# dscripka/openWakeWord

Measured on AMD Instinct MI355X. Metric: real-time audio frames/sec (80 ms frame, 3 wakewords), whole job; real-time streams = value/12.5, higher is better.
Workload: dtype f32 as 3xf16 split MFMA, fp32 accumulate; 1 GPU; 131072 concurrent 16 kHz streams per GPU x 3 heads (alexa,hey_mycroft,hey_jarvis), 80 ms frames, BASELINE configs[3] per-GPU shard; streams_per_gpu=131072, frame_samples=1280, collective=none, gather=none, rccl_ranks=0, pcm_distribution=Gaussian, RMS 3000, pcm=resident in HBM, kernels=mfma_rr_f16x3, graph=False, vad=off, weights=synthetic seed 1234, step_blocks=1

## Files before the change

openwakeword_amd/csrc/owwhip.hip:

```cpp
#include <hip/hip_runtime.h>

#include <algorithm>
#include <cmath>
#include <cstdio>
#include <cstdlib>
#include <cstring>
#include <ctime>
#include <exception>
#include <mutex>
#include <new>
#include <unordered_map>
#include <dlfcn.h>
#include <string>
#include <vector>

#include "owwhip.h"
#include "owwhip_pack.h"
#include "owwhip_ingest.h"
#include "owwhip_mem.h"
#include "owwhip_masked_host.h"
#include "owwhip_bank_host.h"
#include "owwhip_verifier_host.h"
#include "owwhip_state_host.h"
#include "owwhip_postproc.h"
#include "owwhip_kernels.h"
#include "owwhip_rr.h"
#include "owwhip_hx.h"
#include "owwhip_vad.h"
#include "owwhip_fused.h"
#include "owwhip_state.h"
#include "owwhip_events.h"
#include "owwhip_audio.h"
#include "owwhip_dense.h"
#include "owwhip_dense_hits_host.h"

using namespace owk;
using namespace owp;
using owm::DevBuf;
using owm::PinnedBuf;

namespace {

#define OWW_GUARD_BEGIN try {
#define OWW_GUARD_END                                                                                              \
    } catch (const std::bad_alloc&) { return fail(OWW_ENOMEM, "%s: out of host memory", __func__);                 \
    } catch (const std::exception& e__) { return fail(OWW_ESTATE, "%s: unexpected C++ exception: %s", __func__, e__.what()); \
    } catch (...) { return fail(OWW_ESTATE, "%s: unexpected C++ exception", __func__); }

#define HIPCHK(expr)                                                                         \
    do {                                                                                     \
        hipError_t e__ = (expr);                                                             \
        if (e__ != hipSuccess) return fail(OWW_EHIP, "%s failed: %s", #expr, hipGetErrorString(e__)); \
    } while (0)

struct GuardRange { char* base; size_t reserve, mapped; hipMemGenericAllocationHandle_t hnd; };
std::mutex g_guard_mu;
std::unordered_map<void*, GuardRange> g_guard;
int guard_mode() {
    static const int mode = [] { const char* e = getenv("OWW_GUARD_ALLOC"); return e ? atoi(e) : 0; }();
    return mode;
}
hipError_t guard_alloc(void** p, size_t n, int line) {
    int dev = 0;
    hipError_t e = hipGetDevice(&dev);
    if (e != hipSuccess) return e;
    hipMemAllocationProp prop = {};
    prop.type = hipMemAllocationTypePinned;
    prop.location.type = hipMemLocationTypeDevice;
    prop.location.id = dev;
    size_t gran = 0;
    if ((e = hipMemGetAllocationGranularity(&gran, &prop, hipMemAllocationGranularityMinimum)) != hipSuccess) return e;
    GuardRange g{};
    g.mapped = (std::max<size_t>(n, 1) + gran - 1) / gran * gran;
    g.reserve = g.mapped + 2 * gran;
    void* base = nullptr;
    if ((e = hipMemAddressReserve(&base, g.reserve, gran, nullptr, 0)) != hipSuccess) return e;
    g.base = static_cast<char*>(base);
    if ((e = hipMemCreate(&g.hnd, g.mapped, &prop, 0)) != hipSuccess) { (void)hipMemAddressFree(base, g.reserve); return e; }
    hipMemAccessDesc acc = {};
    acc.location = prop.location;
    acc.flags = hipMemAccessFlagsProtReadWrite;
    if ((e = hipMemMap(g.base + gran, g.mapped, 0, g.hnd, 0)) != hipSuccess ||
        (e = hipMemSetAccess(g.base + gran, g.mapped, &acc, 1)) != hipSuccess) {
        (void)hipMemRelease(g.hnd); (void)hipMemAddressFree(base, g.reserve); return e;
    }
    char* user = guard_mode() == 2 ? g.base + gran : g.base + gran + g.mapped - (n + 15) / 16 * 16;
    fprintf(stderr, "[owwhip guard] line %d: %zu bytes at [%p, %p), mapped [%p, %p)\n", line, n, (void*)user, (void*)(user + n),
            (void*)(g.base + gran), (void*)(g.base + gran + g.mapped));
    std::lock_guard<std::mutex> lk(g_guard_mu);
    g_guard[user] = g;
    *p = user;
    return hipSuccess;
}
hipError_t dev_alloc(void** p, size_t n, int line) {
    if (!guard_mode()) return hipMalloc(p, n);
    return guard_alloc(p, n, line);
}
hipError_t dev_free(void* p) {
    if (!guard_mode() || !p) return hipFree(p);
    GuardRange g;
    {
        std::lock_guard<std::mutex> lk(g_guard_mu);
        auto it = g_guard.find(p);
        if (it == g_guard.end()) return hipFree(p);
        g = it->second;
        g_guard.erase(it);
    }
    (void)hipDeviceSynchronize();
    const size_t gran = (g.reserve - g.mapped) / 2;
    (void)hipMemUnmap(g.base + gran, g.mapped);
    (void)hipMemRelease(g.hnd);
    return hipMemAddressFree(g.base, g.reserve);
}
}

namespace owm {
int dev_alloc_raw(void** p, size_t bytes, int line) { return dev_alloc(p, bytes, line); }
int dev_free_raw(void* p) { return dev_free(p); }
int pinned_alloc_raw(void** p, size_t bytes, unsigned flags) { return hipHostMalloc(p, bytes, flags); }
int pinned_free_raw(void* p) { return hipHostFree(p); }
int event_create_raw(hipEvent_t* e, unsigned flags) { return hipEventCreateWithFlags(e, flags); }
int event_destroy_raw(hipEvent_t e) { return hipEventDestroy(e); }
int stream_create_raw(hipStream_t* s, unsigned flags) { return hipStreamCreateWithFlags(s, flags); }
int stream_destroy_raw(hipStream_t s) { return hipStreamDestroy(s); }
}

namespace {
inline hipError_t herr(int e) { return static_cast<hipError_t>(e); }

hipError_t guard_copy(void* dst, const void* src, size_t n, hipMemcpyKind kind, hipStream_t st) {
    PinnedBuf<char> pin;
    hipError_t e = herr(pin.alloc(n, hipHostMallocDefault));
    if (e != hipSuccess) return e;
    if (kind == hipMemcpyHostToDevice) {
        memcpy(pin, src, n);
        e = hipMemcpyAsync(dst, pin, n, kind, st);
        if (e == hipSuccess) e = hipStreamSynchronize(st);
    } else {
        e = hipMemcpyAsync(pin, src, n, kind, st);
        if (e == hipSuccess) e = hipStreamSynchronize(st);
        if (e == hipSuccess) memcpy(dst, pin, n);
    }
    return e;
}
inline hipError_t copy_async(void* dst, const void* src, size_t n, hipMemcpyKind kind, hipStream_t st) {
    if (guard_mode() && n && (kind == hipMemcpyHostToDevice || kind == hipMemcpyDeviceToHost)) return guard_copy(dst, src, n, kind, st);
    return hipMemcpyAsync(dst, src, n, kind, st);
}
inline hipError_t copy_sync(void* dst, const void* src, size_t n, hipMemcpyKind kind) {
    if (guard_mode() && n && (kind == hipMemcpyHostToDevice || kind == hipMemcpyDeviceToHost)) return guard_copy(dst, src, n, kind, nullptr);
    const hipError_t e = hipMemcpy(dst, src, n, kind);
    return e != hipSuccess || kind != hipMemcpyHostToDevice ? e : hipStreamSynchronize(nullptr);
}

constexpr int kSmallLaunchWgs = 2 * 256;
constexpr int kResidentBMinGroups = 8192;
constexpr int kResidentBWgs = 256;

struct FastGroup : HeadGroup {
    DevBuf<NetDesc> d_nets;
    const float* d_w1pk = nullptr;
    const float* d_b1cat = nullptr;
    const float* d_w1hx = nullptr;
    std::vector<owh::HeadHxNet> hx_net;
};

owh::HeadHxNet make_hx_net(const NetHost& n, int ht, const HxNetPack& p, const float* img, const float* b3, int hx_efeat) {
    const int HP = 16 * ht;
    const float* pd = img + p.pad;
    owh::HeadHxNet o{};
    o.w2hx = img + p.w2; o.b1 = pd; o.ln1g = pd + HP; o.ln1b = pd + 2 * HP; o.b2 = pd + 3 * HP; o.ln2g = pd + 4 * HP; o.ln2b = pd + 5 * HP;
    if (ht == 4) { o.w3 = pd + 6 * HP; o.b3 = b3 ? b3 : pd + 7 * HP; }
    else { o.b3 = pd + 6 * HP; o.w3hx = img + p.w3; o.u3 = std::ldexp(1.0f, -p.e3); }
    o.has_ln = n.has_ln; o.role = n.role; o.head = n.head; o.out_col = n.out_col;
    o.hidden = n.hidden; o.inv_hidden = 1.0f / (float)n.hidden;
    o.u1 = std::ldexp(1.0f, -(hx_efeat + p.e1) + (n.has_ln ? 0 : p.eh)); o.u2 = std::ldexp(1.0f, -(p.e2 + p.eh));
    o.n_out = n.n_out; o.final_act = n.final_act;
    return o;
}

struct EventRec { owm::Event a, b; int cls = 0; };

}

struct oww_ctx : PackIn {
    owm::Stream stream, up_stream, down_stream;
    oww_config cfg{};
    int S = 0, Spad = 0, kmax = 1, TR = 16, NL = 0;
    bool committed = false;
    const int* state_len = kStateLenRr;
    ~oww_ctx();
    DevBuf<float> d_w;
    const float *d_hann = nullptr, *d_taps = nullptr;
    const int* d_mstart = nullptr;
    const int* d_meloff = nullptr; const unsigned* d_meldst = nullptr;
    const float* d_conv[20] = {};
    const float* d_scale[20] = {};
    const float* d_shift[20] = {};
    DevBuf<NetDesc> d_allnets;
    std::vector<FastGroup> groups;
    std::vector<int> generic_nets;
    std::vector<int> rnn_nets;
    int generic_hmax = 0;
    int generic_spw = 0;
    DevBuf<float> d_state[N_STATE], d_tmpl[N_STATE];
    DevBuf<float> d_xA, d_xB, d_xC, d_xD;
    DevBuf<float> d_mel, d_feat, d_emb, d_raw, d_scores, d_ring;
    struct IngestSlot {
        DevBuf<int16_t> d_pcm; DevBuf<float> d_scores; PinnedBuf<float> h_scores;
        DevBuf<char> d_mix;
        PinnedBuf<uint8_t> h_on;
        owm::Event up, done, down;
        bool busy = false;
    } slot[2];
    struct EventBuf {
        DevBuf<oww_event> d_rec; DevBuf<int> d_count; DevBuf<float> d_snap;
        DevBuf<int16_t> d_asnap;
        PinnedBuf<oww_event> h_rec; PinnedBuf<int> h_count;
    };
    int evt_cap = 0, evt_rows = 0;
    DevBuf<float> d_evt_thr; float evt_bank_thr = 0.5f;
    DevBuf<int> d_evblock; int evt_blocks = 0;
    EventBuf evt_sync, evt_slot[2];
    const EventBuf* evt_cur = nullptr;
    int aud_ring = 0, aud_evt = 0;
    DevBuf<int16_t> d_aring;
    DevBuf<uint32_t> d_acount;
    DevBuf<int16_t> d_aout; DevBuf<int> d_aids; DevBuf<uint32_t> d_acnt;

    uint64_t n_submit = 0, n_collect = 0;
    DevBuf<float> d_featinit, d_dbg;
    DevBuf<long long> d_prof;
    int prof_block = -1;
    DevBuf<uint32_t> d_nfeat, d_npred, d_nvad;
    DevBuf<float> d_vadring, d_vadin; float vad_threshold = 0.f;
    bool vad = false;
    const float *d_vad_hann = nullptr, *d_vad_encw = nullptr, *d_vad_encb = nullptr, *d_vad_lstmw = nullptr, *d_vad_lstmb = nullptr, *d_vad_wd = nullptr;
    float vad_bd = 0.f, vad_gain = 50.f;
    DevBuf<float> d_vadx, d_vadhc, d_vadlast;
    DevBuf<int16_t> d_tail, d_pcm;
    DevBuf<int16_t> d_long;
    DevBuf<float> d_callmax;
    PinnedBuf<int> h_range;
    int* d_range = nullptr;
    DevBuf<char> d_rs;
    std::vector<float> rs_taps;
    struct Ingest {
        bool ready = false, mixed = false;
        owi::Table tab;
        DevBuf<float> d_taps;
        DevBuf<int16_t> d_hist;
        DevBuf<int16_t> d_out;
        DevBuf<char> d_in;
        DevBuf<uint8_t> d_on;
        DevBuf<IngestClass> d_table;
        DevBuf<uint32_t> d_cls;
        DevBuf<int> d_newcls;
    } ing;
    DevBuf<uint8_t> d_on;
    DevBuf<int> d_lists; PinnedBuf<int> h_lists[2]; owm::Event lists_ev[2]; unsigned lists_turn = 0;
    int k_last = 1;
    float hx_absmax[20] = {};
    std::vector<int16_t> cal_user;
    int small_wgs = kSmallLaunchWgs, small_wgs_heads = kSmallLaunchWgs;
    int resident_b = -1, resident_b_wgs = kResidentBWgs;
    float hx_selftest_err = 0.f, hx_selftest_ref = 0.f, hx_selftest_score_err = 0.f;
    bool fuse = false;
    DevBuf<float> d_verw, d_verb, d_verthr; DevBuf<int> d_verT;
    int ver_stride = 0, n_verifiers = 0;
    std::vector<int> ver_T;
    bool post_in_heads = false;
    DevBuf<float> d_save;
    DevBuf<int> d_ids;
    DevBuf<int> d_patience;
    DevBuf<float> d_threshold;
    int debounce_frames = 0;
    void* comm = nullptr; int comm_rank = 0, comm_world = 1;
    bool timing = false;
    std::vector<EventRec> ev;
    size_t ev_used = 0;
    double t_ms[OWW_N_KERNEL_CLASSES] = {};
    int64_t t_n[OWW_N_KERNEL_CLASSES] = {};
    bool want_graph = false;
    hipGraph_t graph = nullptr;
    hipGraphExec_t graph_exec = nullptr;
    struct BankHead {
        bool live = false;
        int T = 0, hidden = 0, has_ln = 0, ht = 4, patience = 0;
        float threshold = NAN;
        DevBuf<float> d_img;
        size_t w1_bytes = 0;
        owh::BankHeadDev dev{};
    };
    int bank_K = 0, bank_cap = 0;
    std::vector<BankHead> bank;
    std::vector<int> bank_sub;
    DevBuf<int> d_bank_sub, d_bank_idx;
    DevBuf<float> d_bank_raw, d_bank_scores, d_bank_ring;
    DevBuf<uint32_t> d_bank_npred;
    DevBuf<owh::BankHeadDev> d_bank_heads; DevBuf<int> d_bank_pat; DevBuf<float> d_bank_thr;
    DevBuf<owh::BankTile> d_bank_tiles; DevBuf<int> d_bank_entries;
    owb::Route bank_rt;
    int vpool_cap = 0;
    int vpool_stride = 0;
    std::vector<int> vpool_T;
    DevBuf<float> d_vpool_w, d_vpool_b;
    std::vector<int> vasg_fix, vasg_bank;
    std::vector<float> vthr_fix, vthr_bank;
    long long vasg_n = 0;
    std::vector<float> ver_thr;
    DevBuf<SvEntry> d_svlist; int sv_n = 0;
    DevBuf<unsigned long long> d_sv_eval;
    bool st_ready = false;
    std::vector<ows::FlatSection> st_flat;
    std::vector<ows::GroupSection> st_group;
    bool st_levels[4] = {};
    DevBuf<ows::FlatSection> d_st_flat;
    uint32_t st_record_words = 0, st_flat_quads = 0;
    uint64_t st_fp = 0;
    DevBuf<int> d_st_items;
    DevBuf<uint32_t> d_st_stage;
};

namespace {

struct StepArgs {
    const uint8_t* on = nullptr;
    bool lists = false;
    const int* gl[5] = {};
    int gn[5] = {};
    const int16_t* fused_pcm = nullptr;
    bool post_in_heads = false;
    const float* mel = nullptr;
    bool dbg = false;
};

StepArgs step_args(const oww_ctx* h) { StepArgs a; a.dbg = h->d_dbg != nullptr; return a; }

int flush_events(oww_ctx* h) {
    if (!h->ev_used) return 0;
    HIPCHK(hipStreamSynchronize(h->stream));
    for (size_t i = 0; i < h->ev_used; ++i) {
        float ms = 0.f;
        HIPCHK(hipEventElapsedTime(&ms, h->ev[i].a, h->ev[i].b));
        h->t_ms[h->ev[i].cls] += ms;
        h->t_n[h->ev[i].cls] += 1;
    }
    h->ev_used = 0;
    return 0;
}

struct Timed {
    oww_ctx* h;
    EventRec* r = nullptr;
    Timed(oww_ctx* h_, int cls) : h(h_) {
        if (!h->timing) return;
        if (h->ev_used == h->ev.size()) {
            if (h->ev.size() >= 8192) { flush_events(h); }
            else {
                EventRec e;
                if (e.a.create(hipEventDefault) || e.b.create(hipEventDefault)) return;
                h->ev.push_back(std::move(e));
            }
        }
        r = &h->ev[h->ev_used++];
        r->cls = cls;
        (void)hipEventRecord(r->a, h->stream);
    }
    ~Timed() { if (r) (void)hipEventRecord(r->b, h->stream); }
};

template <class K>
int set_lds(K kernel, int bytes) {
    HIPCHK(hipFuncSetAttribute(reinterpret_cast<const void*>(kernel), hipFuncAttributeMaxDynamicSharedMemorySize, bytes));
    return 0;
}

template <bool MFMA>
int run_cnn_t(oww_ctx* h, const StepArgs& a, int n_active, int mel_stride, int mel_off) {
    hipStream_t st = h->stream;
    const bool dbg = a.dbg;
    int off = 0;
    int dbg_off[20];
    for (int l = 0; l < 20; ++l) { dbg_off[l] = off; off += kLayerOut[l][0] * kLayerOut[l][1] * kLayerOut[l][2]; }
    {
        StageAParams p{};
        p.mel = a.mel ? a.mel : h->d_mel; p.mel_stride = mel_stride; p.mel_off = mel_off;
        p.hist_mel = h->d_state[0]; p.hist2 = h->d_state[1];
        p.w0 = h->d_conv[0]; p.w1 = h->d_conv[1]; p.w2 = h->d_conv[2];
        for (int i = 0; i < 3; ++i) { p.scale[i] = h->d_scale[i]; p.shift[i] = h->d_shift[i]; p.dbg_off[i] = dbg_off[i]; }
        p.xout = h->d_xA; p.dbg = dbg ? h->d_dbg : nullptr; p.dbg_stride = DBG_FLOATS;
        Timed t(h, 1);
        hipLaunchKernelGGL(stageA_kernel<MFMA>, dim3(n_active), dim3(CfgA::NT), CfgA::LDS_BYTES, st, p);
    }
    auto fill = [&](StageParams& p, const float* xin, float* xout, int first_layer, int sb, int sd) {
        p.xin = xin; p.xout = xout; p.hist_b = h->d_state[sb]; p.hist_d = h->d_state[sd];
        for (int i = 0; i < 4; ++i) {
            p.w[i] = h->d_conv[first_layer + i]; p.scale[i] = h->d_scale[first_layer + i];
            p.shift[i] = h->d_shift[first_layer + i]; p.dbg_off[i] = dbg_off[first_layer + i];
        }
        p.dbg = dbg ? h->d_dbg : nullptr; p.dbg_stride = DBG_FLOATS;
        p.prof = h->d_prof ? h->d_prof + (first_layer / 4) * 256 : nullptr;
        p.prof_block = h->prof_block;
    };
    {
        StageParams p{}; fill(p, h->d_xA, h->d_xB, 3, 2, 3);
        Timed t(h, 2);
        hipLaunchKernelGGL((stage_kernel<CfgB, MFMA, false>), dim3((n_active + CfgB::B - 1) / CfgB::B), dim3(CfgB::NT), CfgB::LDS_BYTES, st, p);
    }
    {
        StageParams p{}; fill(p, h->d_xB, h->d_xC, 7, 4, 5);
        Timed t(h, 3);
        hipLaunchKernelGGL((stage_kernel<CfgC, MFMA, false>), dim3((n_active + CfgC::B - 1) / CfgC::B), dim3(CfgC::NT), CfgC::LDS_BYTES, st, p);
    }
    {
        StageParams p{}; fill(p, h->d_xC, h->d_xD, 11, 6, 7);
        Timed t(h, 4);
        hipLaunchKernelGGL((stage_kernel<CfgD, MFMA, false>), dim3((n_active + CfgD::B - 1) / CfgD::B), dim3(CfgD::NT), CfgD::LDS_BYTES, st, p);
    }
    {
        StageParams p{}; fill(p, h->d_xD, nullptr, 15, 8, 9);
        p.hist19 = h->d_state[10]; p.w19 = h->d_conv[19]; p.feat = h->d_feat; p.emb = h->d_emb; p.nfeat = h->d_nfeat; p.TR = h->TR;
        p.dbg_off[4] = dbg_off[19];
        Timed t(h, 5);
        hipLaunchKernelGGL((stage_kernel<CfgE, MFMA, true>), dim3((n_active + CfgE::B - 1) / CfgE::B), dim3(CfgE::NT), CfgE::LDS_BYTES, st, p);
    }
    HIPCHK(hipGetLastError());
    return 0;
}

template <class CR, class CH, int WG, bool LAST, bool DBG, bool HX>
void launch_rstage(oww_ctx* h, const owr::RStageParams& p, int cls) {
    hipStream_t st = h->stream;
    Timed t(h, cls);
    const int nwg = (p.n_groups + WG - 1) / WG;
    if constexpr (HX && !DBG && std::is_same<CH, owh::HB>::value) {
        const bool resident = p.glist == nullptr && p.n_groups > 0 && (h->resident_b < 0 ? p.n_groups >= kResidentBMinGroups : h->resident_b != 0);
        if (resident) {
            const int grid = std::max(1, std::min(h->resident_b_wgs, (p.n_groups + owh::RES_B_WG - 1) / owh::RES_B_WG));
            hipLaunchKernelGGL((owh::hstage_kernel<CH, LAST, false, owh::RES_B_WG, 1>), dim3(grid), dim3(64 * owh::RES_B_WG), owh::RES_B_LDS_BYTES, st, p);
            return;
        }
    }
    if (HX && !DBG && nwg <= h->small_wgs) hipLaunchKernelGGL((owh::hstage_kernel<CH, LAST, false, WG, 3>), dim3(nwg), dim3(64 * WG), 0, st, p);
    else if (HX) hipLaunchKernelGGL((owh::hstage_kernel<CH, LAST, DBG, WG>), dim3(nwg), dim3(64 * WG), 0, st, p);
    else hipLaunchKernelGGL((owr::rstage_kernel<CR, LAST, DBG>), dim3((p.n_groups + 3) / 4), dim3(256), 0, st, p);
}

template <bool DBG, bool HX>
int run_cnn_rr(oww_ctx* h, const StepArgs& a, int n_active, int mel_stride, int mel_off) {
    using namespace owr;
    hipStream_t st = h->stream;
    int off = 0, dbg_off[20];
    for (int l = 0; l < 20; ++l) { dbg_off[l] = off; off += kLayerOut[l][0] * kLayerOut[l][1] * kLayerOut[l][2]; }
    {
        RAParams p{};
        p.mel = a.mel ? a.mel : h->d_mel; p.mel_stride = mel_stride; p.mel_off = mel_off;
        p.hist_mel = h->d_state[0]; p.hist2 = h->d_state[1];
        p.w0 = h->d_conv[0]; p.w1 = h->d_conv[1]; p.w2 = h->d_conv[2];
        for (int i = 0; i < 3; ++i) { p.scale[i] = h->d_scale[i]; p.shift[i] = h->d_shift[i]; p.dbg_off[i] = dbg_off[i]; }
        p.xout = h->d_xA; p.n_streams = n_active; p.S = h->Spad;
        p.dbg = DBG ? h->d_dbg : nullptr; p.dbg_stride = DBG_FLOATS;
        for (int i = 0; i < 3; ++i) { p.clampv[i] = -0.4f * ldexpf(1.f, h->hx_e[i]); p.dbg_mul[i] = ldexpf(1.f, -h->hx_e[i]); }
        p.xmul = ldexpf(1.f, h->hx_xexp[0]);
        p.range_flag = HX ? h->d_range : nullptr;
        p.stream_on = a.on;
        const int grid = std::min((n_active + 3) / 4, 768);
        Timed t(h, 1);
        if (HX && a.fused_pcm) {
            owf::MelAParams q{};
            q.a = p; q.a.mel = nullptr; q.a.n_streams = h->S;
            q.pcm = a.fused_pcm; q.tail = h->d_tail; q.nfeat = h->d_nfeat; q.hann = h->d_hann; q.mel_start = h->d_mstart; q.mel_taps = h->d_taps; q.mel_off = h->d_meloff; q.mel_dst = h->d_meldst;
            q.mel_out = h->cfg.debug_layers ? h->d_mel : nullptr;
            const int per_cu = std::max(1, std::min(12 / owf::FA_WG, 163840 / owf::FA_LDS_BYTES));
            const int g2 = std::max(1, std::min((q.a.n_streams + owf::FA_WG - 1) / owf::FA_WG, 256 * per_cu));
            hipLaunchKernelGGL(owf::hmelA_kernel<DBG>, dim3(g2), dim3(64 * owf::FA_WG), owf::FA_LDS_BYTES, st, q);
        }
        else if (HX) hipLaunchKernelGGL(owh::hstageA_kernel<DBG>, dim3(std::min((n_active + 3) / 4, 256 * OWH_WPS_A)), dim3(256), 0, st, p);
        else hipLaunchKernelGGL(rstageA_kernel<DBG>, dim3(grid), dim3(256), 0, st, p);
    }
    auto fill = [&](const float* xin, float* xout, int first_layer, int sb, int sd, int spt) {
        RStageParams p{};
        p.xin = xin; p.xout = xout; p.hist_b = h->d_state[sb]; p.hist_d = h->d_state[sd];
        for (int i = 0; i < 4; ++i) {
            p.w[i] = h->d_conv[first_layer + i]; p.scale[i] = h->d_scale[first_layer + i];
            p.shift[i] = h->d_shift[first_layer + i]; p.dbg_off[i] = dbg_off[first_layer + i];
            p.clampv[i] = -0.4f * ldexpf(1.f, h->hx_e[first_layer + i]); p.dbg_mul[i] = ldexpf(1.f, -h->hx_e[first_layer + i]);
        }
        p.dbg_mul[4] = ldexpf(1.f, -h->hx_e[19]);
        p.xmul = ldexpf(1.f, h->hx_xexp[first_layer / 4 + 1]);
        p.emb_mul = ldexpf(1.f, -h->hx_e[19]);
        p.n_groups = (n_active + spt - 1) / spt; p.S = h->Spad;
        p.dbg = DBG ? h->d_dbg : nullptr; p.dbg_stride = DBG_FLOATS;
        p.range_flag = HX ? h->d_range : nullptr;
        p.stream_on = a.on;
        if (HX && a.lists) {
            const int k = spt == 1 ? 0 : spt == 2 ? 1 : spt == 4 ? 2 : 3;
            p.glist = a.gl[k]; p.n_groups = a.gn[k];
        }
        return p;
    };
    launch_rstage<RB, owh::HB, OWH_WG_B, false, DBG, HX>(h, fill(h->d_xA, h->d_xB, 3, 2, 3, RB::SPT), 2);
    launch_rstage<RC, owh::HC, OWH_WG_C, false, DBG, HX>(h, fill(h->d_xB, h->d_xC, 7, 4, 5, RC::SPT), 3);
    launch_rstage<RD, owh::HD, OWH_WG_D, false, DBG, HX>(h, fill(h->d_xC, h->d_xD, 11, 6, 7, RD::SPT), 4);
    RStageParams pe = fill(h->d_xD, nullptr, 15, 8, 9, RE::SPT);
    pe.hist19 = h->d_state[10]; pe.w19 = h->d_conv[19]; pe.feat = h->d_feat; pe.emb = h->d_emb; pe.nfeat = h->d_nfeat; pe.TR = h->TR;
    pe.dbg_off[4] = dbg_off[19];
    launch_rstage<RE, owh::HE, OWH_WG_E, true, DBG, HX>(h, pe, 5);
    HIPCHK(hipGetLastError());
    return 0;
}

int run_cnn(oww_ctx* h, const StepArgs& a, int n_active, int mel_stride, int mel_off) {
    n_active = std::min(h->Spad, (n_active + 7) / 8 * 8);
    if (h->hx) return a.dbg ? run_cnn_rr<true, true>(h, a, n_active, mel_stride, mel_off) : run_cnn_rr<false, true>(h, a, n_active, mel_stride, mel_off);
    if (h->rr) return a.dbg ? run_cnn_rr<true, false>(h, a, n_active, mel_stride, mel_off) : run_cnn_rr<false, false>(h, a, n_active, mel_stride, mel_off);
    return h->mfma ? run_cnn_t<true>(h, a, n_active, mel_stride, mel_off) : run_cnn_t<false>(h, a, n_active, mel_stride, mel_off);
}

owq::Rules post_rules(const oww_ctx* h) { return {h->d_patience, h->d_threshold, h->debounce_frames}; }
owq::Rules bank_post_rules(const oww_ctx* h) { return {h->d_bank_pat, h->d_bank_thr, h->debounce_frames}; }
owq::Gate post_gate(const oww_ctx* h) { return {h->d_vadring, h->d_nvad, h->vad_threshold}; }

int heads_lds_bytes(int NH) { return (HD_SB * 100 + 2 * HD_SB * (NH + 4) + HD_SB * HD_MAXNETS) * 4; }

void launch_generic_heads(oww_ctx* h, const HeadParams& p, int n_active, int nb, int ne, hipStream_t st) {
    const int hs = (std::max(h->generic_hmax, 1) + 3) & ~3;
    const bool big = h->generic_hmax <= 128 && (h->generic_spw == 16 || (h->generic_spw == 0 && n_active >= GH_BIG_STREAMS));
    if (big) hipLaunchKernelGGL((heads_generic_kernel<16, 2, 2>), dim3((n_active + 31) / 32), dim3(128), gh_lds_bytes(16, 2, hs), st, p, nb, ne, hs);
    else hipLaunchKernelGGL((heads_generic_kernel<4, 4>), dim3((n_active + 15) / 16), dim3(256), gh_lds_bytes(4, 4, hs), st, p, nb, ne, hs);
}

int run_heads(oww_ctx* h, const StepArgs& a, int n_active, bool accumulate_max, const float* ext, int only_head, float* raw_out, int force_generic) {
    hipStream_t st = h->stream;
    Timed t(h, 6);
    HeadParams base{};
    base.feat = ext ? ext : h->d_feat; base.ext = ext ? 1 : 0; base.TR = h->TR; base.nfeat = h->d_nfeat;
    base.raw = raw_out; base.NL = h->NL; base.S = n_active; base.accumulate_max = accumulate_max ? 1 : 0;
    base.stream_on = ext ? nullptr : a.on;
    const bool fast_ok = h->mfma && !force_generic;
    if (fast_ok) {
        for (auto& g : h->groups) {
            if (only_head >= 0) {
                bool has = false;
                for (int ni : g.nets) has |= h->nets[ni].head == only_head;
                if (!has) continue;
            }
            if (h->hx) {
                owh::HeadHxParams q{};
                q.feat = base.feat; q.ext = base.ext; q.TR = base.TR; q.T = g.T; q.nfeat = base.nfeat; q.w1hx = g.d_w1hx;
                q.raw = raw_out; q.NL = h->NL; q.S = n_active; q.accumulate_max = base.accumulate_max;
                q.range_flag = h->d_range; q.stream_on = a.on;
                if (a.lists && !ext) { q.ids = a.gl[0]; q.n_ids = a.gn[0]; }
                const int n_pos = q.ids ? q.n_ids : q.S;
                if (a.post_in_heads) {
                    owh::HeadHxPost& pp = q.post;
                    pp.enabled = 1; pp.scores = h->d_scores; pp.ring = h->d_ring; pp.npred = h->d_npred; pp.nfeat = h->d_nfeat;
                    pp.rules = post_rules(h); pp.gate = post_gate(h);
                }
                for (int i = 0; i < g.n_nets; ++i) q.net[i] = g.hx_net[i];
                q.fscale = std::ldexp(1.0f, h->hx_efeat);
                const dim3 grid((n_pos + 32 * owh::HX_WG - 1) / (32 * owh::HX_WG)), block(64 * owh::HX_WG);
                const bool deep = (int)grid.x <= h->small_wgs_heads;
                const int nn = std::min(g.n_nets, 4);
                const int lds = 0;
                if (g.ht == 8) {
                    if (nn == 1 && !deep) hipLaunchKernelGGL((owh::heads_hx_kernel<1, owh::HX_NBUF, owh::HX_WG, 8>), grid, block, lds, st, q);
                    else if (nn == 1) hipLaunchKernelGGL((owh::heads_hx_kernel<1, owh::HeadsDeep<2>::NBUF, owh::HX_WG, 8>), grid, block, lds, st, q);
                    else if (!deep) hipLaunchKernelGGL((owh::heads_hx_kernel<2, owh::HX_NBUF, owh::HX_WG, 8>), grid, block, lds, st, q);
                    else hipLaunchKernelGGL((owh::heads_hx_kernel<2, owh::HeadsDeep<4>::NBUF, owh::HX_WG, 8>), grid, block, lds, st, q);
                    continue;
                }
                switch (nn * 2 + (deep ? 1 : 0)) {
                    case 2: hipLaunchKernelGGL(owh::heads_hx_kernel<1>, grid, block, lds, st, q); break;
                    case 3: hipLaunchKernelGGL((owh::heads_hx_kernel<1, owh::HeadsDeep<1>::NBUF>), grid, block, lds, st, q); break;
                    case 4: hipLaunchKernelGGL(owh::heads_hx_kernel<2>, grid, block, lds, st, q); break;
                    case 5: hipLaunchKernelGGL((owh::heads_hx_kernel<2, owh::HeadsDeep<2>::NBUF>), grid, block, lds, st, q); break;
                    case 6: hipLaunchKernelGGL(owh::heads_hx_kernel<3>, grid, block, lds, st, q); break;
                    case 7: hipLaunchKernelGGL((owh::heads_hx_kernel<3, owh::HeadsDeep<3>::NBUF>), grid, block, lds, st, q); break;
                    case 8: hipLaunchKernelGGL(owh::heads_hx_kernel<4>, grid, block, lds, st, q); break;
                    default: hipLaunchKernelGGL((owh::heads_hx_kernel<4, owh::HeadsDeep<4>::NBUF>), grid, block, lds, st, q); break;
                }
                continue;
            }
            HeadParams p = base;
            p.nets = g.d_nets; p.n_nets = g.n_nets; p.T = g.T; p.NH = g.NH; p.w1pk = g.d_w1pk; p.b1cat = g.d_b1cat;
            hipLaunchKernelGGL(heads64_kernel, dim3((n_active + HD_SB - 1) / HD_SB), dim3(HD_NT), heads_lds_bytes(g.NH), st, p);
        }
    }
    if (!fast_ok) {
        HeadParams p = base;
        p.nets = h->d_allnets; p.n_nets = (int)h->nets.size();
        int nb = 0, ne = (int)h->nets.size();
        if (only_head >= 0) { nb = h->head_nets[only_head].first; ne = h->head_nets[only_head].second; }
        launch_generic_heads(h, p, n_active, nb, ne, st);
    } else if (!h->generic_nets.empty()) {
// ... 611 lines not shown
    if (!r.tiles.empty()) HIPCHK(copy_sync(h->d_bank_tiles, r.tiles.data(), r.tiles.size() * sizeof(owh::BankTile), hipMemcpyHostToDevice));
    if (!r.entries.empty()) HIPCHK(copy_sync(h->d_bank_entries, r.entries.data(), r.entries.size() * sizeof(int), hipMemcpyHostToDevice));
    if (h->graph_exec) { (void)hipGraphExecDestroy(h->graph_exec); h->graph_exec = nullptr; }
    return 0;
}

int sv_rebuild(oww_ctx* h) {
    const std::vector<SvEntry> list = owsv::sv_list(h->S, h->NL, h->bank_K, h->vasg_fix, h->vthr_fix, h->vasg_bank, h->vthr_bank, h->vpool_T, h->ver_T,
                                                    h->ver_thr, h->vasg_n);
    if (!list.empty()) HIPCHK(copy_sync(h->d_svlist, list.data(), list.size() * sizeof(SvEntry), hipMemcpyHostToDevice));
    h->sv_n = (int)list.size();
    const unsigned long long zero = 0;
    HIPCHK(copy_sync(h->d_sv_eval, &zero, sizeof zero, hipMemcpyHostToDevice));
    if (h->graph_exec) { (void)hipGraphExecDestroy(h->graph_exec); h->graph_exec = nullptr; }
    return 0;
}

int sv_drop_bank(oww_ctx* h, const std::vector<int>& slots) {
    if (h->vpool_cap == 0) return 0;
    bool any = false;
    for (int at : slots)
        if (h->vasg_bank[at] != OWW_VERIFIER_DEFAULT) { h->vasg_bank[at] = OWW_VERIFIER_DEFAULT; --h->vasg_n; any = true; }
    return any ? sv_rebuild(h) : 0;
}

void comm_release(oww_ctx* h) {
    if (h->comm && g_rccl.CommDestroy) (void)g_rccl.CommDestroy(h->comm);
    h->comm = nullptr; h->comm_rank = 0; h->comm_world = 1;
}

}

oww_ctx::~oww_ctx() {
    for (hipStream_t st : {stream.get(), up_stream.get(), down_stream.get()})
        if (st) (void)hipStreamSynchronize(st);
    comm_release(this);
    if (graph_exec) (void)hipGraphExecDestroy(graph_exec);
    if (graph) (void)hipGraphDestroy(graph);
}

namespace {

int bind_weights(oww_ctx* h, const HostBuf& hb, const WeightOff& off) {
    HIPCHK(herr(h->d_w.alloc(hb.data.size())));
    HIPCHK(copy_sync(h->d_w, hb.data.data(), hb.data.size() * sizeof(float), hipMemcpyHostToDevice));
    const float* w = h->d_w;
    h->d_hann = w + off.hann; h->d_mstart = reinterpret_cast<const int*>(w + off.start); h->d_taps = w + off.taps;
    h->d_meloff = reinterpret_cast<const int*>(w + off.meloff); h->d_meldst = reinterpret_cast<const unsigned*>(w + off.meldst);
    if (h->vad) {
        h->d_vad_hann = w + off.vhann; h->d_vad_encw = w + off.vencw; h->d_vad_encb = w + off.vencb;
        h->d_vad_lstmw = w + off.vlw; h->d_vad_lstmb = w + off.vlb; h->d_vad_wd = w + off.vwd;
    }
    for (int l = 0; l < 20; ++l) {
        h->d_conv[l] = w + off.conv[l];
        h->d_scale[l] = l < 19 ? w + off.scale[l] : nullptr;
        h->d_shift[l] = l < 19 ? w + off.shift[l] : nullptr;
    }
    auto make_desc = [&](int ni, int hid_off) {
        const NetHost& n = h->nets[ni];
        const WeightOff::Net& o = off.net[ni];
        NetDesc d{};
        d.hidden = n.hidden; d.n_out = n.n_out; d.has_ln = n.has_ln; d.final_act = n.final_act; d.T = n.T;
        d.head = n.head; d.role = n.role; d.out_col = n.out_col; d.hid_off = hid_off;
        if (n.rnn) { d.rnn = w + o.rnn; return d; }
        d.w1 = w + o.w1; d.b1 = w + o.b1;
        d.ln1g = n.has_ln ? w + o.ln1g : nullptr; d.ln1b = n.has_ln ? w + o.ln1b : nullptr;
        d.n_blocks = n.n_blocks;
        d.blocks = n.n_blocks > 0 ? w + o.blocks : nullptr;
        d.w2 = n.n_blocks > 0 ? w + o.w2 : nullptr; d.b2 = n.n_blocks > 0 ? w + o.b2 : nullptr;
        d.ln2g = n.has_ln && n.n_blocks > 0 ? w + o.ln2g : nullptr; d.ln2b = n.has_ln && n.n_blocks > 0 ? w + o.ln2b : nullptr;
        d.w3 = w + o.w3; d.b3 = w + o.b3;
        d.w2pk = n.hidden == 64 && n.n_blocks == 1 ? w + o.w2pk : nullptr;
        return d;
    };
    if (!h->nets.empty()) {
        std::vector<NetDesc> all;
        for (size_t ni = 0; ni < h->nets.size(); ++ni) all.push_back(make_desc((int)ni, 0));
        HIPCHK(herr(h->d_allnets.alloc(all.size())));
        HIPCHK(copy_sync(h->d_allnets, all.data(), all.size() * sizeof(NetDesc), hipMemcpyHostToDevice));
    }
    for (size_t gi = 0; gi < h->groups.size(); ++gi) {
        FastGroup& g = h->groups[gi];
        const WeightOff::Group& go = off.group[gi];
        std::vector<NetDesc> ds;
        for (int i = 0; i < g.n_nets; ++i) ds.push_back(make_desc(g.nets[i], 64 * i));
        HIPCHK(herr(g.d_nets.alloc(ds.size())));
        HIPCHK(copy_sync(g.d_nets, ds.data(), ds.size() * sizeof(NetDesc), hipMemcpyHostToDevice));
        g.d_w1pk = w + go.w1pk; g.d_b1cat = w + go.b1cat;
        if (!h->hx) continue;
        g.d_w1hx = w + go.w1hx;
        for (int i = 0; i < g.n_nets; ++i)
            g.hx_net.push_back(make_hx_net(h->nets[g.nets[i]], g.ht, go.net[i], w, g.ht == 4 ? w + off.net[g.nets[i]].b3 : nullptr, h->hx_efeat));
    }
    return 0;
}

int alloc_range_flag(oww_ctx* h) {
    void* dp = nullptr;
    HIPCHK(herr(h->h_range.alloc(16, hipHostMallocMapped)));
    h->h_range[0] = 0; h->h_range[1] = -1;
    HIPCHK(hipHostGetDevicePointer(&dp, h->h_range, 0));
    h->d_range = (int*)dp;
    return 0;
}

int alloc_state(oww_ctx* h) {
    const size_t SP = h->Spad;
    for (int a = 0; a < N_STATE; ++a) {
        if (int rc = dalloc(h->stream, h->d_state[a], SP * h->state_len[a])) return rc;
        if (int rc = dalloc(h->stream, h->d_tmpl[a], (size_t)h->state_len[a] * (h->rr ? kStateSpgRr[a] : 1))) return rc;
    }
    const int* xlen = h->rr ? kXLenRr : kXLenLds;
    DevBuf<float>* x[4] = {&h->d_xA, &h->d_xB, &h->d_xC, &h->d_xD};
    for (int i = 0; i < 4; ++i) if (int rc = dalloc(h->stream, *x[i], SP * xlen[i])) return rc;
    if (int rc = dalloc(h->stream, h->d_mel, SP * 8 * h->kmax * 32)) return rc;
    if (int rc = dalloc(h->stream, h->d_feat, SP * h->TR * 96)) return rc;
    if (int rc = dalloc(h->stream, h->d_emb, SP * 96)) return rc;
    if (int rc = dalloc(h->stream, h->d_raw, SP * std::max(h->NL, 1))) return rc;
    if (int rc = dalloc(h->stream, h->d_scores, SP * std::max(h->NL, 1))) return rc;
    if (int rc = dalloc(h->stream, h->d_ring, SP * std::max(h->NL, 1) * OWW_SCORE_RING)) return rc;
    if (int rc = dalloc(h->stream, h->d_featinit, (size_t)h->TR * 96)) return rc;
    if (int rc = dalloc(h->stream, h->d_nfeat, SP)) return rc;
    if (int rc = dalloc(h->stream, h->d_npred, SP)) return rc;
    if (int rc = dalloc(h->stream, h->d_vadring, SP * owq::kVadRing)) return rc;
    if (int rc = dalloc(h->stream, h->d_nvad, SP)) return rc;
    if (int rc = dalloc(h->stream, h->d_vadin, SP)) return rc;
    if (h->vad) {
        const size_t G = (SP + 15) / 16;
        if (int rc = dalloc(h->stream, h->d_vadx, G * 4 * 1024)) return rc;
        if (int rc = dalloc(h->stream, h->d_vadhc, G * 4096)) return rc;
        if (int rc = dalloc(h->stream, h->d_vadlast, SP)) return rc;
    }
    if (int rc = dalloc(h->stream, h->d_tail, SP * 480)) return rc;
    if (int rc = dalloc(h->stream, h->d_pcm, (size_t)h->S * OWW_CHUNK * h->kmax)) return rc;
    if (int rc = dalloc(h->stream, h->d_patience, (size_t)std::max(h->NL, 1))) return rc;
    if (int rc = dalloc(h->stream, h->d_threshold, (size_t)std::max(h->NL, 1))) return rc;
    {
        std::vector<float> nanv(std::max(h->NL, 1), NAN);
        HIPCHK(copy_async(h->d_threshold, nanv.data(), nanv.size() * sizeof(float), hipMemcpyHostToDevice, h->stream));
    }
    if (h->cfg.debug_layers) if (int rc = dalloc(h->stream, h->d_dbg, SP * DBG_FLOATS)) return rc;
    if (const char* e = getenv("OWW_PROF_BLOCK")) { h->prof_block = atoi(e); if (int rc = dalloc(h->stream, h->d_prof, (size_t)4 * 256)) return rc; }
    return 0;
}

int set_kernel_lds(oww_ctx* h) {
    int rc = 0;
    auto lds = [&rc](auto kernel, int bytes) { if (!rc) rc = set_lds(kernel, bytes); };
    for (const auto& g : h->groups) if (g.ht == 4) lds(heads64_kernel, heads_lds_bytes(g.NH));
    if (!h->rnn_nets.empty()) lds(heads_rnn_kernel<RNN_SPW>, (int)rnn_lds_bytes(RNN_TMAX));
    if (h->vad) lds(owv::vad_front_kernel, owv::V_LDS_BYTES);
    lds(owf::hmelA_kernel<false>, owf::FA_LDS_BYTES); lds(owf::hmelA_kernel<true>, owf::FA_LDS_BYTES);
    lds(owh::hstage_kernel<owh::HB, false, false, owh::RES_B_WG, 1>, owh::RES_B_LDS_BYTES);
    lds(stageA_kernel<true>, CfgA::LDS_BYTES); lds(stageA_kernel<false>, CfgA::LDS_BYTES);
    lds(stage_kernel<CfgB, true, false>, CfgB::LDS_BYTES); lds(stage_kernel<CfgB, false, false>, CfgB::LDS_BYTES);
    lds(stage_kernel<CfgC, true, false>, CfgC::LDS_BYTES); lds(stage_kernel<CfgC, false, false>, CfgC::LDS_BYTES);
    lds(stage_kernel<CfgD, true, false>, CfgD::LDS_BYTES); lds(stage_kernel<CfgD, false, false>, CfgD::LDS_BYTES);
    lds(stage_kernel<CfgE, true, true>, CfgE::LDS_BYTES); lds(stage_kernel<CfgE, false, true>, CfgE::LDS_BYTES);
    return rc;
}

int derive_reset_state(oww_ctx* h, const HxCalib& cal, CommitClock& clk) {
    const size_t SP = h->Spad;
    const int warm = std::min<int>(32, (int)SP);
    hipLaunchKernelGGL(fill_kernel, dim3((warm * 256 + 255) / 256), dim3(256), 0, h->stream, h->d_mel, (size_t)warm * 256, 1.0f);
    const StepArgs args{};
    for (int it = 0; it < 12; ++it)
        if (int rc = run_cnn(h, args, warm, 256, 0)) return rc;
    for (int a = 0; a < N_STATE; ++a)
        HIPCHK(copy_async(h->d_tmpl[a], h->d_state[a], (size_t)h->state_len[a] * (h->rr ? kStateSpgRr[a] : 1) * sizeof(float),
                              hipMemcpyDeviceToDevice, h->stream));
    HIPCHK(hipMemsetAsync(h->d_mel, 0, SP * 8 * h->kmax * 32 * sizeof(float), h->stream));
    HIPCHK(hipMemsetAsync(h->d_emb, 0, SP * 96 * sizeof(float), h->stream));
    if (int rc = do_reset(h, nullptr, (int)SP, nullptr)) return rc;
    HIPCHK(hipStreamSynchronize(h->stream));
    clk.lap("warm-up + reset");
    if (int rc = range_check(h, "oww_commit")) return rc;
    if (h->hx && !getenv("OWW_NO_COMMIT_SELFTEST")) {
        if (int rc = selftest_hx(h, cal)) return rc;
        HIPCHK(hipMemsetAsync(h->d_mel, 0, SP * 8 * h->kmax * 32 * sizeof(float), h->stream));
        HIPCHK(hipMemsetAsync(h->d_emb, 0, SP * 96 * sizeof(float), h->stream));
        HIPCHK(hipMemsetAsync(h->d_raw, 0, SP * std::max(h->NL, 1) * sizeof(float), h->stream));
        if (int rc = do_reset(h, nullptr, (int)SP, nullptr)) return rc;
        HIPCHK(hipStreamSynchronize(h->stream));
        clk.lap("self-test replay + reset");
    }
    return 0;
}

int alloc_bank(oww_ctx* h) {
    const size_t SK = (size_t)h->S * h->bank_K;
    if (int rc = dalloc(h->stream, h->d_bank_sub, SK, false)) return rc;
    if (int rc = dalloc(h->stream, h->d_bank_idx, SK)) return rc;
    if (int rc = dalloc(h->stream, h->d_bank_raw, SK)) return rc;
    if (int rc = dalloc(h->stream, h->d_bank_scores, SK)) return rc;
    if (int rc = dalloc(h->stream, h->d_bank_ring, SK * OWW_SCORE_RING)) return rc;
    if (int rc = dalloc(h->stream, h->d_bank_npred, SK)) return rc;
    if (int rc = dalloc(h->stream, h->d_bank_entries, SK)) return rc;
    if (int rc = dalloc(h->stream, h->d_bank_heads, (size_t)h->bank_cap)) return rc;
    if (int rc = dalloc(h->stream, h->d_bank_pat, (size_t)h->bank_cap)) return rc;
    if (int rc = dalloc(h->stream, h->d_bank_thr, (size_t)h->bank_cap, false)) return rc;
    h->bank.clear(); h->bank.resize(h->bank_cap);
    h->bank_sub.assign(SK, -1);
    std::vector<float> nanv(h->bank_cap, NAN);
    HIPCHK(copy_async(h->d_bank_sub, h->bank_sub.data(), SK * sizeof(int), hipMemcpyHostToDevice, h->stream));
    HIPCHK(copy_async(h->d_bank_thr, nanv.data(), nanv.size() * sizeof(float), hipMemcpyHostToDevice, h->stream));
    HIPCHK(hipStreamSynchronize(h->stream));
    return 0;
}

int alloc_verifiers(oww_ctx* h) {
    h->vpool_stride = h->TR * OWW_EMB_DIM;
    if (int rc = dalloc(h->stream, h->d_vpool_w, (size_t)h->vpool_cap * h->vpool_stride)) return rc;
    if (int rc = dalloc(h->stream, h->d_vpool_b, (size_t)h->vpool_cap)) return rc;
    if (int rc = dalloc(h->stream, h->d_svlist, (size_t)h->S * (h->NL + h->bank_K), false)) return rc;
    if (int rc = dalloc(h->stream, h->d_sv_eval, 1)) return rc;
    h->vpool_T.assign(h->vpool_cap, 0);
    h->vasg_fix.assign((size_t)h->S * h->NL, OWW_VERIFIER_DEFAULT);
    h->vthr_fix.assign((size_t)h->S * h->NL, 0.f);
    h->vasg_bank.assign((size_t)h->S * h->bank_K, OWW_VERIFIER_DEFAULT);
    h->vthr_bank.assign((size_t)h->S * h->bank_K, 0.f);
    h->vasg_n = 0; h->sv_n = 0;
    HIPCHK(hipStreamSynchronize(h->stream));
    return 0;
}


int state_layout(oww_ctx* h) {
    if (h->st_ready) return 0;
    h->st_flat.clear(); h->st_group.clear();
    auto flat = [&](void* live, size_t stride, size_t len) { h->st_flat.push_back(ows::FlatSection{static_cast<uint32_t*>(live), (uint32_t)stride, (uint32_t)len, 0, 0}); };
    const bool il = h->hx && owh::kInterleave;
    const size_t NL = (size_t)h->NL, K = (size_t)h->bank_K;
    for (int a = 0; a < N_STATE; ++a)
        if (!h->rr || kStateSpgRr[a] == 1) flat(h->d_state[a], h->state_len[a], h->state_len[a]);
    flat(h->d_tail, 240, 240);
    flat(h->d_feat, (size_t)h->TR * OWW_EMB_DIM, (size_t)h->TR * OWW_EMB_DIM);
    flat(h->d_ring, NL * OWW_SCORE_RING, NL * OWW_SCORE_RING);
    flat(h->d_raw, NL, NL); flat(h->d_scores, NL, NL);
    flat(h->d_nfeat, 1, 1); flat(h->d_npred, 1, 1);
    flat(h->d_vadring, owq::kVadRing, owq::kVadRing); flat(h->d_nvad, 1, 1);
    if (h->vad) flat(h->d_vadlast, 1, 1);
    if (K) { flat(h->d_bank_raw, K, K); flat(h->d_bank_scores, K, K); flat(h->d_bank_npred, K, K); flat(h->d_bank_ring, K * OWW_SCORE_RING, K * OWW_SCORE_RING); }
    const oww_ctx::Ingest& ing = h->ing;
    if (ing.ready && ing.tab.Hpad_max) flat(ing.d_hist, (size_t)ing.tab.Hpad_max / 2, (size_t)ing.tab.Hpad_max / 2);
    if (ing.ready && ing.mixed) flat(ing.d_cls, 1, 1);
    if (audio_on(h)) {
        flat(h->d_aring, owa::ring_words(h->aud_ring), owa::ring_words(h->aud_ring));
        flat(h->d_acount, owa::kCounterWords, owa::kCounterWords);
    }
    for (int a = 0; a < N_STATE; ++a)
        if (h->rr && kStateSpgRr[a] > 1)
            h->st_group.push_back(ows::GroupSection{h->d_state[a], kStateSpgRr[a], il ? 16 / kStateSpgRr[a] : kStateFposRr[a], il, (uint32_t)(h->state_len[a] * kStateSpgRr[a]), 0});
    if (h->vad) h->st_group.push_back(ows::GroupSection{h->d_vadhc, 16, 1, true, 4096, 0});
    ows::Layout L;
    if (int rc = ows::layout(h->st_flat, h->st_group, L)) return rc;
    h->st_flat_quads = L.flat_quads; h->st_record_words = L.record_words;
    for (int lv = 0; lv < 4; ++lv) {
        h->st_levels[lv] = false;
        for (const auto& g : h->st_group) h->st_levels[lv] = h->st_levels[lv] || g.spg == ows::kStateLevels[lv];
    }
    std::vector<ows::HeadPrint> heads;
    for (const auto& hh : h->heads) heads.push_back(ows::HeadPrint{{hh.kind, hh.T, hh.hidden, hh.n_out, hh.has_ln, hh.n_blocks}, {hh.blob.data(), hh.blob.size() * sizeof(float)}});
    const uint64_t fp = ows::fingerprint(h->cfg.use_mfma, il, h->state_len, N_STATE, h->TR, h->NL, h->bank_K, h->vad, h->hx ? h->hx_e : nullptr, h->hx_efeat,
                                         {h->mel_blob.data(), h->mel_blob.size() * sizeof(float)}, {h->emb_blob.data(), h->emb_blob.size() * sizeof(float)}, heads,
                                         {h->vad_blob.data(), h->vad_blob.size() * sizeof(float)});
    h->st_fp = owa::fingerprint(owi::fingerprint(fp, ing.ready, ing.mixed, ing.tab), h->aud_ring);
    if (!h->d_st_flat) HIPCHK(herr(h->d_st_flat.alloc(h->st_flat.size())));
    HIPCHK(copy_sync(h->d_st_flat, h->st_flat.data(), h->st_flat.size() * sizeof(ows::FlatSection), hipMemcpyHostToDevice));
    h->st_ready = true;
    return 0;
}

int state_lists_upload(oww_ctx* h, const std::vector<int>& buf) {
    if (grow(h, h->d_st_items, buf.size()) != hipSuccess) return fail(OWW_ENOMEM, "out of device memory for %zu stream list bytes", buf.size() * sizeof(int));
    HIPCHK(copy_async(h->d_st_items, buf.data(), buf.size() * sizeof(int), hipMemcpyHostToDevice, h->stream));
    return 0;
}

int state_stage(oww_ctx* h, size_t n) {
    const size_t need = n * (size_t)h->st_record_words;
    if (grow(h, h->d_st_stage, need) != hipSuccess) return fail(OWW_ENOMEM, "out of device memory for %zu bytes of stream state records", need * 4);
    return 0;
}

template <bool SCATTER>
int state_xfer(oww_ctx* h, const ows::StateList& L, uint32_t* rec) {
    if (L.n == 0) return 0;
    ows::FlatParams fp{};
    fp.ids = h->d_st_items + L.ids_at; fp.sec = h->d_st_flat; fp.n_sec = (int)h->st_flat.size(); fp.flat_quads = h->st_flat_quads;
    fp.rec = rec; fp.record_words = h->st_record_words; fp.record_bytes = h->st_record_words * 4;
    fp.fp_lo = (uint32_t)h->st_fp; fp.fp_hi = (uint32_t)(h->st_fp >> 32);
    hipLaunchKernelGGL(ows::state_flat_kernel<SCATTER>, dim3(L.n, (h->st_flat_quads + 255) / 256), dim3(256), 0, h->stream, fp);
    HIPCHK(hipGetLastError());
    for (const auto& g : h->st_group) {
        int lv = 0;
        while (ows::kStateLevels[lv] != g.spg) ++lv;
        if (L.n_groups[lv] == 0) continue;
        ows::GroupParams gp{};
        const int R = g.ppr >= 4 ? 1 : 4 / g.ppr;
        gp.live = reinterpret_cast<uint32_t*>(g.live); gp.block_words = g.block_words; gp.items = h->d_st_items + L.items_at[lv];
        gp.n_chunks = (int)(g.block_words / (16 * R)); gp.rec = rec; gp.record_words = h->st_record_words; gp.off = g.off;
        const dim3 grid(L.n_groups[lv], (gp.n_chunks + 63) / 64);
#define OWS_GO(SPG, PPR, IL) hipLaunchKernelGGL((ows::state_group_kernel<SPG, PPR, IL, SCATTER>), grid, dim3(64), 0, h->stream, gp)
        if (g.il) {
            if (g.spg == 2) OWS_GO(2, 8, true); else if (g.spg == 4) OWS_GO(4, 4, true); else if (g.spg == 8) OWS_GO(8, 2, true); else OWS_GO(16, 1, true);
// ... 426 lines not shown
int oww_abi_version(void) { return OWW_ABI_VERSION; }
#ifndef OWW_SRC_SHA16
#define OWW_SRC_SHA16 "unknown"
#endif
const char* oww_build_info(void) { return "src=" OWW_SRC_SHA16 " arch=gfx950"; }
const char* oww_last_error(void) { return g_err.c_str(); }

int oww_create(const oww_config* cfg, oww_ctx** out) {
    OWW_GUARD_BEGIN
    if (!cfg || !out) return fail(OWW_EINVAL, "oww_create: null argument");
    if (cfg->n_streams < 1) return fail(OWW_EINVAL, "oww_create: n_streams must be >= 1");
    int ndev = 0;
    HIPCHK(hipGetDeviceCount(&ndev));
    if (cfg->device < 0 || cfg->device >= ndev) return fail(OWW_EINVAL, "oww_create: device %d of %d", cfg->device, ndev);
    HIPCHK(hipSetDevice(cfg->device));
    oww_ctx* h = new (std::nothrow) oww_ctx();
    if (!h) return fail(OWW_ENOMEM, "oww_create: out of host memory");
    h->cfg = *cfg;
    h->S = cfg->n_streams;
    h->Spad = (h->S + 31) / 32 * 32;
    h->kmax = std::max(1, cfg->max_chunks);
    h->mfma = cfg->use_mfma != 0;
    h->rr = cfg->use_mfma == 1 || cfg->use_mfma == 3;
    h->hx = cfg->use_mfma == 3;
    h->state_len = h->rr ? kStateLenRr : kStateLenLds;
    if (cfg->stream) h->stream.borrow(reinterpret_cast<hipStream_t>(cfg->stream));
    else if (const int e = h->stream.create(hipStreamNonBlocking)) { delete h; return fail(OWW_EHIP, "hipStreamCreate: %s", hipGetErrorString(herr(e))); }
    *out = h;
    return OWW_OK;
    OWW_GUARD_END
}

int oww_destroy(oww_ctx* h) {
    OWW_GUARD_BEGIN
    if (!h) return OWW_OK;
    (void)hipSetDevice(h->cfg.device);
    delete h;
    return OWW_OK;
    OWW_GUARD_END
}

int oww_load_mel(oww_ctx* h, const void* blob, size_t nbytes) {
    OWW_GUARD_BEGIN
    if (!h || !blob) return fail(OWW_EINVAL, "oww_load_mel: null argument");
    if (h->committed) return fail(OWW_ESTATE, "weights already committed");
    return parse_mel_blob(blob, nbytes, h->mel_blob);
    OWW_GUARD_END
}

int oww_load_embedding(oww_ctx* h, const void* blob, size_t nbytes) {
    OWW_GUARD_BEGIN
    if (!h || !blob) return fail(OWW_EINVAL, "oww_load_embedding: null argument");
    if (h->committed) return fail(OWW_ESTATE, "weights already committed");
    return parse_embedding_blob(blob, nbytes, h->emb_blob);
    OWW_GUARD_END
}

int oww_add_head(oww_ctx* h, const void* blob, size_t nbytes) {
    OWW_GUARD_BEGIN
    if (!h || !blob || nbytes < 32) return fail(OWW_EINVAL, "oww_add_head: bad argument");
    if (h->committed) return fail(OWW_ESTATE, "weights already committed");
    if ((int)h->heads.size() >= OWW_MAX_HEADS) return fail(OWW_EINVAL, "too many heads");
    HeadHost hh{};
    if (int rc = parse_head_blob("oww_add_head", blob, nbytes, 120, hh)) return rc;
    h->heads.push_back(std::move(hh));
    return (int)h->heads.size() - 1;
    OWW_GUARD_END
}

int oww_load_vad(oww_ctx* h, const void* blob, size_t nbytes) {
    OWW_GUARD_BEGIN
    if (!h || !blob) return fail(OWW_EINVAL, "oww_load_vad: null argument");
    if (h->committed) return fail(OWW_ESTATE, "weights already committed");
    return parse_vad_blob(blob, nbytes, h->vad_blob);
    OWW_GUARD_END
}

int oww_set_calibration(oww_ctx* h, const int16_t* pcm, int32_t n_streams, int32_t n_frames) {
    OWW_GUARD_BEGIN
    if (!h) return fail(OWW_EINVAL, "oww_set_calibration: null handle");
    if (h->committed) return fail(OWW_ESTATE, "oww_set_calibration: call before oww_commit");
    h->cal_user.clear();
    if (!pcm || n_streams < 1 || n_frames < 1) return OWW_OK;
    const size_t seg = (size_t)CAL_T * OWW_CHUNK;
    const int per = (n_frames + CAL_T - 1) / CAL_T;
    const size_t n_seg = std::min<size_t>((size_t)n_streams * per, (size_t)(CAL_MAX_BATCHES - 1) * CAL_NP);
    h->cal_user.assign(n_seg * seg, 0);
    for (size_t k = 0; k < n_seg; ++k) {
        const size_t s = k / per, part = k % per;
        const size_t first = part * seg, n = std::min(seg, (size_t)n_frames * OWW_CHUNK - first);
        memcpy(&h->cal_user[k * seg], pcm + s * (size_t)n_frames * OWW_CHUNK + first, n * sizeof(int16_t));
    }
    return OWW_OK;
    OWW_GUARD_END
}

int oww_calibration_info(oww_ctx* h, float absmax[20], int32_t exps[21], int32_t* n_probe_streams, float selftest[3]) {
    OWW_GUARD_BEGIN
    if (!h || !h->committed) return fail(OWW_ESTATE, "oww_calibration_info: handle not committed");
    if (!h->hx) return fail(OWW_ESTATE, "oww_calibration_info: only the fp16-split family (use_mfma = 3) calibrates");
    if (absmax) memcpy(absmax, h->hx_absmax, sizeof h->hx_absmax);
    if (exps) { for (int l = 0; l < 20; ++l) exps[l] = h->hx_e[l]; exps[20] = h->hx_efeat; }
    if (n_probe_streams) *n_probe_streams = CAL_NP + (int32_t)(h->cal_user.size() / ((size_t)CAL_T * OWW_CHUNK));
    if (selftest) { selftest[0] = h->hx_selftest_err; selftest[1] = h->hx_selftest_ref; selftest[2] = h->hx_selftest_score_err; }
    return OWW_OK;
    OWW_GUARD_END
}

int oww_n_labels(const oww_ctx* h) { return h ? h->NL : 0; }

int oww_commit(oww_ctx* h) {
    OWW_GUARD_BEGIN
    if (!h) return fail(OWW_EINVAL, "null handle");
    if (h->committed) return fail(OWW_ESTATE, "already committed");
    if (h->mel_blob.empty() || h->emb_blob.empty()) return fail(OWW_ESTATE, "mel and embedding weights must be loaded before commit");
    HIPCHK(hipSetDevice(h->cfg.device));
    h->feature_ring = h->cfg.feature_ring;
    if (int rc = build_nets(*h, h->NL, h->TR, h->generic_hmax)) return rc;
    if (h->evt_rows > h->TR)
        return fail(OWW_EINVAL, "oww_events_configure: feature_rows = %d exceeds the handle's feature ring (%d rows)", h->evt_rows, h->TR);
    if (int rc = owa::commit_check(h->aud_evt, h->evt_cap)) return rc;
    CommitClock clk(h->hx ? "f16-split" : "family");
    HxCalib cal;
    if (h->hx) {
        if (int rc = calibrate_hx(h, cal)) return rc;
        h->probe_emb = cal.ref_emb; h->probe_nb = cal.nb;
        clk.lap("calibration (total)");
        if (getenv("OWW_DEBUG_CALIB"))
            for (int l = 0; l < 20; ++l) fprintf(stderr, "calib layer %2d: max|a| %-12.5g e_in %4d e_out %4d\n", l, h->hx_absmax[l], h->hx_ein[l], h->hx_e[l]);
    }
    HostBuf hb;
    WeightOff off;
    HeadGroups hg;
    h->no_wide_heads = getenv("OWW_NO_WIDE_HEADS") != nullptr;
    if (int rc = pack_mel_tables(*h, hb, off)) return rc;
    if (int rc = pack_cnn(*h, hb, off)) return rc;
    pack_net_arrays(*h, hb, off);
    if (int rc = pack_head_groups(*h, hg, hb, off)) return rc;
    h->groups.clear();
    for (const HeadGroup& g : hg.groups) h->groups.push_back(FastGroup{g});
    h->generic_nets = hg.generic_nets; h->rnn_nets = hg.rnn_nets;
    h->vad = !h->vad_blob.empty();
    if (int rc = pack_vad(*h, hb, off, h->vad_gain, h->vad_bd)) return rc;
    clk.lap("weight packing (host)");
    if (int rc = bind_weights(h, hb, off)) return rc;
    if (int rc = alloc_range_flag(h)) return rc;
    clk.lap("weight upload");
    if (int rc = alloc_state(h)) return rc;
    h->fuse = h->hx && !getenv("OWW_NO_FUSE");
    if (const char* e = getenv("OWW_SMALL_WGS")) h->small_wgs = atoi(e);
    if (const char* e = getenv("OWW_SMALL_WGS_HEADS")) h->small_wgs_heads = atoi(e);
    if (const char* e = getenv("OWW_RESIDENT_B")) h->resident_b = strcmp(e, "auto") == 0 ? -1 : (atoi(e) != 0 ? 1 : 0);
    if (const char* e = getenv("OWW_RESIDENT_B_WGS")) h->resident_b_wgs = std::max(1, atoi(e));
    if (const char* e = getenv("OWW_GENERIC_SPW")) { const int v = atoi(e); h->generic_spw = v == 4 || v == 16 ? v : 0; }
    h->post_in_heads = h->fuse && h->groups.size() == 1 && h->groups[0].ht == 4 && h->generic_nets.empty() && h->rnn_nets.empty() && h->NL > 0;
    if (int rc = set_kernel_lds(h)) return rc;
    clk.lap("state allocation");
    if (int rc = derive_reset_state(h, cal, clk)) return rc;
    if (h->bank_K > 0) if (int rc = alloc_bank(h)) return rc;
    if (h->vpool_cap > 0) if (int rc = alloc_verifiers(h)) return rc;
    if (audio_on(h)) if (int rc = alloc_audio(h)) return rc;
    if (events_on(h)) if (int rc = alloc_events(h)) return rc;
    h->committed = true;
    return OWW_OK;
    OWW_GUARD_END
}

int oww_reset(oww_ctx* h, const int32_t* stream_ids, int32_t n, const float* init_features) {
    OWW_GUARD_BEGIN
    if (!h || !h->committed) return fail(OWW_ESTATE, "oww_reset: handle not committed");
    HIPCHK(hipSetDevice(h->cfg.device));
    const float* d_init = nullptr;
    if (init_features) {
        HIPCHK(copy_async(h->d_featinit, init_features, (size_t)h->TR * 96 * sizeof(float), hipMemcpyHostToDevice, h->stream));
        d_init = h->d_featinit;
    }
    if (!stream_ids) {
        if (int rc = do_reset(h, nullptr, h->Spad, d_init)) return rc;
    } else {
        if (n < 1) return OWW_OK;
        for (int i = 0; i < n; ++i)
            if (stream_ids[i] < 0 || stream_ids[i] >= h->S) return fail(OWW_EINVAL, "oww_reset: stream id %d out of range", stream_ids[i]);
        if (int rc = upload_ids(h, stream_ids, n)) return rc;
        if (int rc = do_reset(h, h->d_ids, n, d_init)) return rc;
    }
    if (h->ing.ready && h->ing.tab.Hpad_max) {
        hipLaunchKernelGGL(ingest_hist_reset_kernel, dim3(stream_ids ? n : h->S), dim3(64), 0, h->stream, h->ing.d_hist, h->ing.tab.Hpad_max,
                           stream_ids ? h->d_ids : nullptr, stream_ids ? n : h->S);
        HIPCHK(hipGetLastError());
    }
    if (audio_on(h)) if (int rc = audio_reset(h, stream_ids ? (const int*)h->d_ids : nullptr, n)) return rc;
    std::vector<int> slots;
    if (h->bank_K > 0) {
        if (!stream_ids) for (int i = 0; i < h->S * h->bank_K; ++i) slots.push_back(i);
        else for (int i = 0; i < n; ++i) for (int k = 0; k < h->bank_K; ++k) slots.push_back(stream_ids[i] * h->bank_K + k);
        if (int rc = bank_clear(h, slots)) return rc;
    }
    HIPCHK(hipStreamSynchronize(h->stream));
    return OWW_OK;
    OWW_GUARD_END
}

int oww_set_postproc(oww_ctx* h, const int32_t* patience, const float* threshold, int32_t debounce_frames) {
    OWW_GUARD_BEGIN
    if (!h || !h->committed) return fail(OWW_ESTATE, "oww_set_postproc: handle not committed");
    HIPCHK(hipSetDevice(h->cfg.device));
    std::vector<int> pat(std::max(h->NL, 1), 0);
    std::vector<float> thr(std::max(h->NL, 1), NAN);
    if (patience) for (int i = 0; i < h->NL; ++i) pat[i] = patience[i];
    if (threshold) for (int i = 0; i < h->NL; ++i) thr[i] = threshold[i];
    HIPCHK(copy_async(h->d_patience, pat.data(), pat.size() * sizeof(int), hipMemcpyHostToDevice, h->stream));
    HIPCHK(copy_async(h->d_threshold, thr.data(), thr.size() * sizeof(float), hipMemcpyHostToDevice, h->stream));
    HIPCHK(hipStreamSynchronize(h->stream));
    h->debounce_frames = debounce_frames;
    if (h->graph_exec) { (void)hipGraphExecDestroy(h->graph_exec); h->graph_exec = nullptr; }
    return OWW_OK;
    OWW_GUARD_END
}

int oww_step(oww_ctx* h, const int16_t* pcm, int pcm_on_device, int32_t n_chunks, float* scores, int scores_on_device) {
    OWW_GUARD_BEGIN
    if (!h || !h->committed) return fail(OWW_ESTATE, "oww_step: handle not committed");
    if (!pcm) return fail(OWW_EINVAL, "oww_step: pcm is null");
    if (n_chunks < 1 || n_chunks > OWW_MAX_CALL_CHUNKS) return fail(OWW_EINVAL, "oww_step: n_chunks=%d outside [1,%d]", n_chunks, OWW_MAX_CALL_CHUNKS);
    if (int rc = range_check(h, "oww_step")) return rc;
    HIPCHK(hipSetDevice(h->cfg.device));
    h->k_last = n_chunks;
    const StepArgs a = step_args(h);
    const size_t n_pcm = (size_t)h->S * OWW_CHUNK * n_chunks;
    if (n_chunks > h->kmax) {
        const int16_t* d_call = pcm;
        if (!pcm_on_device) {
            if (grow(h, h->d_long, n_pcm) != hipSuccess) return fail(OWW_ENOMEM, "oww_step: out of device memory for a call of %d chunks", n_chunks);
            HIPCHK(copy_async(h->d_long, pcm, n_pcm * sizeof(int16_t), hipMemcpyHostToDevice, h->stream));
            d_call = h->d_long;
        }
        if (int rc = launch_step_long(h, a, d_call, n_chunks)) return rc;
        if (audio_on(h)) if (int rc = launch_audio_append(h, a, d_call, n_chunks)) return rc;
        if (events_on(h)) { if (int rc = launch_events(h, a, h->evt_sync)) return rc; h->evt_cur = &h->evt_sync; }
        return deliver_scores(h, scores, scores_on_device, !scores_on_device || !pcm_on_device, "oww_step");
    }
    const bool graphable = h->want_graph && n_chunks == 1 && !h->timing;
    const int16_t* d_pcm = pcm;
    if (!pcm_on_device || graphable) {
        HIPCHK(copy_async(h->d_pcm, pcm, n_pcm * sizeof(int16_t), pcm_on_device ? hipMemcpyDeviceToDevice : hipMemcpyHostToDevice, h->stream));
        d_pcm = h->d_pcm;
    }
    if (graphable) {
        if (!h->graph_exec) {
            HIPCHK(hipStreamBeginCapture(h->stream, hipStreamCaptureModeThreadLocal));
            const int rc = launch_step(h, a, h->d_pcm, 1);
            hipGraph_t g = nullptr;
            const hipError_t e = hipStreamEndCapture(h->stream, &g);
            if (rc) return rc;
            if (e != hipSuccess) return fail(OWW_EHIP, "hipStreamEndCapture: %s", hipGetErrorString(e));
            if (h->graph) (void)hipGraphDestroy(h->graph);
            h->graph = g;
            HIPCHK(hipGraphInstantiate(&h->graph_exec, h->graph, nullptr, nullptr, 0));
        }
        HIPCHK(hipGraphLaunch(h->graph_exec, h->stream));
    } else {
        if (int rc = launch_step(h, a, d_pcm, n_chunks)) return rc;
    }
    if (audio_on(h)) if (int rc = launch_audio_append(h, a, d_pcm, n_chunks)) return rc;
    if (events_on(h)) { if (int rc = launch_events(h, a, h->evt_sync)) return rc; h->evt_cur = &h->evt_sync; }
    return deliver_scores(h, scores, scores_on_device, scores && !scores_on_device, "oww_step");
    OWW_GUARD_END
}

int oww_step_masked(oww_ctx* h, const int16_t* pcm, int pcm_on_device, const uint8_t* stream_on, int stream_on_on_device,
                    float* scores, int scores_on_device) {
    OWW_GUARD_BEGIN
    if (!h || !h->committed) return fail(OWW_ESTATE, "oww_step_masked: handle not committed");
    if (!pcm || !stream_on) return fail(OWW_EINVAL, "oww_step_masked: null argument");
    if (!h->rr) return fail(OWW_EINVAL, "oww_step_masked: needs the register-resident kernel families (use_mfma = 3 or 1)");
    if (int rc = range_check(h, "oww_step_masked")) return rc;
    HIPCHK(hipSetDevice(h->cfg.device));
    h->k_last = 1;
    if (int rc = ensure_mask(h)) return rc;
    HIPCHK(copy_async(h->d_on, stream_on, h->S, stream_on_on_device ? hipMemcpyDeviceToDevice : hipMemcpyHostToDevice, h->stream));
    const int16_t* d_pcm = pcm;
    if (!pcm_on_device || (reinterpret_cast<uintptr_t>(pcm) & 15)) {
        HIPCHK(copy_async(h->d_pcm, pcm, (size_t)h->S * OWW_CHUNK * sizeof(int16_t),
                              pcm_on_device ? hipMemcpyDeviceToDevice : hipMemcpyHostToDevice, h->stream));
        d_pcm = h->d_pcm;
    }
    StepArgs a = step_args(h);
    a.on = h->d_on;
    int n_act = -1;
    if (!stream_on_on_device) {
        n_act = build_active_lists(h, stream_on, a);
        if (n_act < -1) return n_act + 100;
    }
    if (n_act != 0)
        if (int rc = launch_step(h, a, d_pcm, 1)) return rc;
    if (audio_on(h)) if (int rc = launch_audio_append(h, a, d_pcm, 1, n_act != 0)) return rc;
    if (events_on(h)) { if (int rc = launch_events(h, a, h->evt_sync, n_act != 0)) return rc; h->evt_cur = &h->evt_sync; }
    return deliver_scores(h, scores, scores_on_device, scores && !scores_on_device, "oww_step_masked");
    OWW_GUARD_END
}

static int ensure_ingest(oww_ctx* h) {
    if (h->up_stream) return 0;
    HIPCHK(herr(h->up_stream.create(hipStreamNonBlocking)));
    HIPCHK(herr(h->down_stream.create(hipStreamNonBlocking)));
    const size_t n_sc = (size_t)h->S * std::max(h->NL, 1);
// ... 1551 lines not shown
```

openwakeword_amd/csrc/owwhip_hx.h:

```cpp
#pragma once
#include <type_traits>
#include <utility>
#include "owwhip_bank_host.h"
#include "owwhip_layout.h"
#include "owwhip_postproc.h"
#include "owwhip_rr.h"

namespace owh {

using owr::f32x4;
typedef _Float16 f16x8 __attribute__((ext_vector_type(8)));

constexpr float WUNSCALE = 1.0f / 256.0f;

__device__ __forceinline__ float act1(float x, float cl) {
    return fmaxf(fmaxf(0.2f * x, x), cl);
}
template <bool ACT, bool HALF>
__device__ __forceinline__ f32x4 act_t(const f32x4 v, float cl) {
    if (!ACT) return HALF ? f32x4{v[0], v[1], 0.f, 0.f} : v;
    if (HALF) return f32x4{act1(v[0], cl), act1(v[1], cl), 0.f, 0.f};
    return f32x4{act1(v[0], cl), act1(v[1], cl), act1(v[2], cl), act1(v[3], cl)};
}
template <bool HALF>
// ... 101 lines not shown
    Op o;
    o.h = __builtin_bit_cast(f16x8, u32x4{hp[0], hp[1], 0u, 0u});
    o.l = __builtin_bit_cast(f16x8, u32x4{hp[0], hp[1], lp[0], lp[1]});
    return o;
}

template <int NCT, bool HALF = false, bool REM2 = false>
__device__ __forceinline__ void to_ops(const f32x4 (&t)[NCT], Op (&o)[(NCT + 1) / 2]) {
    constexpr int KS = (NCT + 1) / 2;
    constexpr int NP_LAST = (NCT % 2 ? 2 : 4) - (HALF ? 1 : 0);
    static_assert(!REM2 || (NCT % 2 == 1 && !HALF), "REM2: an odd, full last channel tile");
#pragma unroll
    for (int k = 0; k < KS; ++k) {
        const f32x4 b = 2 * k + 1 < NCT ? t[2 * k + 1] : f32x4{0.f, 0.f, 0.f, 0.f};
        if (REM2 && k == KS - 1) o[k] = split_dup(t[2 * k]);
        else if (k == KS - 1 && NP_LAST < 4) o[k] = split_some<NP_LAST>(t[2 * k], b);
        else o[k] = split_pair(t[2 * k], b);
        pin_op(o[k]);
    }
}

template <int NCT, bool HALF>
__device__ __forceinline__ void load_tile_h(f32x4 (&t)[NCT], const float* __restrict__ base, int lane) {
#pragma unroll
    for (int ct = 0; ct < NCT; ++ct)
#pragma unroll
        for (int e = 0; e < 4; ++e) {
            if (HALF && ct == NCT - 1 && e >= 2) t[ct][e] = 0.f;
            else t[ct][e] = base[(ct * 4 + e) * 64 + lane];
        }
}
template <int NCT, bool HALF>
__device__ __forceinline__ void store_tile_h(const f32x4 (&t)[NCT], float* __restrict__ base, int lane) {
#pragma unroll
    for (int ct = 0; ct < NCT; ++ct)
#pragma unroll
        for (int e = 0; e < 4; ++e) {
            if (HALF && ct == NCT - 1 && e >= 2) continue;
            base[(ct * 4 + e) * 64 + lane] = t[ct][e];
        }
}

template <int F> __device__ __forceinline__ int tile_stream(int pos) { return kInterleave ? pos % (16 / F) : pos / F; }
template <int F> __device__ __forceinline__ int tile_mel(int pos) { return kInterleave ? pos / (16 / F) : pos % F; }
template <int F> __device__ __forceinline__ int tile_pos(int stream, int mel) { return kInterleave ? mel * (16 / F) + stream : stream * F + mel; }
template <int N> __device__ __forceinline__ float dpp_shr_zero(float x) {
    return __builtin_bit_cast(float, __builtin_amdgcn_update_dpp(0, __builtin_bit_cast(int, x), 0x110 + N, 0xf, 0xf, true));
}
template <int N> __device__ __forceinline__ float dpp_shl_zero(float x) {
    return __builtin_bit_cast(float, __builtin_amdgcn_update_dpp(0, __builtin_bit_cast(int, x), 0x100 + N, 0xf, 0xf, true));
}
#ifndef OWH_UNPAIRED_MIN_F
#define OWH_UNPAIRED_MIN_F 8
#endif
template <int F> __device__ __forceinline__ float unpaired(float s) {
    if (F >= OWH_UNPAIRED_MIN_F) asm("" : "+v"(s));
    return s;
}

template <int NCT, int F, int C>
__device__ __forceinline__ void dump_tile_ht(const f32x4 (&t)[NCT], float* __restrict__ dbg, size_t stride, int off, int s_first,
                                             int row, int S, int lane, float mul) {
    const int pos = lane & 15, j = lane >> 4;
    const int sp = tile_stream<F>(pos), f = tile_mel<F>(pos), s = s_first + sp;
    if (s >= S) return;
#pragma unroll
    for (int ct = 0; ct < NCT; ++ct)
#pragma unroll
        for (int e = 0; e < 4; ++e) {
            int c = ct * 16 + 4 * j + e;
            if (C % 16 == 8 && ct == NCT - 1) c = e < 2 ? ct * 16 + 2 * j + e : C;
            if (c < C) dbg[(size_t)s * stride + off + (row * F + f) * C + c] = t[ct][e] * mul;
        }
}

__device__ __forceinline__ f16x8 lds_h(const float* buf, int blk, int lane) {
    return *reinterpret_cast<const f16x8*>(buf + (blk * 64 + lane) * 4);
}

#ifndef OWH_WG
#define OWH_WG 4
#endif
#ifndef OWH_WG_B
#define OWH_WG_B OWH_WG
#endif
#ifndef OWH_WG_C
#define OWH_WG_C OWH_WG
#endif
#ifndef OWH_WG_D
#define OWH_WG_D OWH_WG
#endif
#ifndef OWH_WG_E
#define OWH_WG_E OWH_WG
#endif
#ifndef OWH_WPS_A
#define OWH_WPS_A 3
#endif
#ifndef OWH_WPS_B
#define OWH_WPS_B 3
#endif
#ifndef OWH_WPS_D
#define OWH_WPS_D 2
#endif
#ifndef OWH_WPS_E
#define OWH_WPS_E 3
#endif
#ifndef OWH_RC_RP
#define OWH_RC_RP 4
#endif
#ifndef OWH_RB_RP
#define OWH_RB_RP 4
#endif
using HB = owr::RCfg<24, 48, 4, 16, 1, 2, OWH_RB_RP, OWH_WPS_B>;
using HC = owr::RCfg<48, 72, 4, 8, 2, 2, OWH_RC_RP, OWH_WPS_C>;
using HD = owr::RCfg<72, 96, 2, 4, 1, 2, 2, OWH_WPS_D>;
using HE = owr::RCfg<96, 96, 2, 2, 2, 2, 2, OWH_WPS_E>;

#define OWH_MFMA(a, b, c) __builtin_amdgcn_mfma_f32_16x16x32_f16(a, b, c, 0, 0, 0)

#ifndef OWH_PRICE_HANDOVER
#define OWH_PRICE_HANDOVER 0
#endif
template <bool ON> __device__ __forceinline__ int price_alias(int i) { return ON ? (i & 511) : i; }

template <int N> __device__ __forceinline__ void wait_vmcnt() {
    static_assert(N >= 0 && N < 64, "vmcnt is a 6-bit field");
    __builtin_amdgcn_s_waitcnt((N & 0xF) | ((N >> 4) << 14) | (0x7 << 4) | (0xF << 8));
    asm volatile("" ::: "memory");
}
template <int NS> struct WRing { float* s[5]; };
template <int MAX> __device__ __forceinline__ void wait_vmcnt_of(int n) {
    if (n >= MAX) wait_vmcnt<MAX>();
    else if constexpr (MAX > 0) wait_vmcnt_of<MAX - 1>(n);
}
template <int NBLK, int WG>
__device__ __forceinline__ void issue_chunk_uniform(const float* __restrict__ gsrc, float* ldst, int wave, int lane) {
    const unsigned voff = lane * 4;
#pragma unroll
    for (int u = 0; u < (NBLK + WG - 1) / WG; ++u) {
        const int i = min(u * WG + wave, NBLK - 1);
        const float* base = owr::uniform_ptr(gsrc + i * 256);
        __builtin_amdgcn_global_load_lds((const __attribute__((address_space(1))) void*)(base + voff),
                                         (__attribute__((address_space(3))) void*)(ldst + i * 256), 16, 0, 0);
    }
}
template <int NS, int NBLK, int WG>
__device__ __forceinline__ void ring_issue(const float* __restrict__ gsrc, float* ldst, int wave, int lane) {
    if constexpr (NS == 2) owr::issue_chunk<NBLK, WG>(gsrc, ldst, wave, lane);
    else issue_chunk_uniform<NBLK, WG>(gsrc, ldst, wave, lane);
}
template <int NS, int CH, int NBLK, int NCTO, int NEXT_NBLK, int WG>
__device__ __forceinline__ const float* ring_begin(const WRing<NS>& r, int oct, const float* __restrict__ w, const float* __restrict__ w_next,
                                                   int wave, int lane) {
    if constexpr (NS == 1) {
        int z = 0;
        asm volatile("" : "+s"(z));
        return r.s[CH / NCTO] + oct * NBLK * 256 + z;
    } else {
    constexpr int P = NS - 1;
    const int c = oct + P;
    float* dst = r.s[(CH + oct + P) % NS];
    if (c < NCTO) ring_issue<NS, NBLK, WG>(w + (size_t)c * NBLK * 256, dst, wave, lane);
    else if (NEXT_NBLK > 0 && c - NCTO < P) ring_issue<NS, (NEXT_NBLK > 0 ? NEXT_NBLK : 1), WG>(w_next + (size_t)(c - NCTO) * NEXT_NBLK * 256, dst, wave, lane);
    return r.s[(CH + oct) % NS];
    }
}
template <int NS, int NBLK, int NCTO, int NEXT_NBLK, int WG>
__device__ __forceinline__ void ring_end(int oct) {
    if (NS == 1 || !(oct + 1 < NCTO || NEXT_NBLK > 0)) return;
    if constexpr (NS == 1) {}
    else if constexpr (NS == 2) owr::chunk_sync();
    else {
        constexpr int P = NS - 1, A = (NBLK + WG - 1) / WG, B = NEXT_NBLK > 0 ? ((NEXT_NBLK > 0 ? NEXT_NBLK : 1) + WG - 1) / WG : 0;
        int n = 0;
#pragma unroll
        for (int c = oct + 2; c <= oct + P; ++c) n += c < NCTO ? A : ((NEXT_NBLK > 0 && c - NCTO < P) ? B : 0);
        wait_vmcnt_of<(P - 1) * (A > B ? A : B)>(n);
        asm volatile("s_waitcnt lgkmcnt(0)\n\ts_barrier" ::: "memory");
    }
}

#ifndef OWH_APIPE_B
#define OWH_APIPE_B 0
#endif
#ifndef OWH_APIPE_C
#define OWH_APIPE_C 3
#endif
#ifndef OWH_APIPE_D
#define OWH_APIPE_D 0
#endif
#ifndef OWH_APIPE_E
#define OWH_APIPE_E 1
#endif
struct APair { f16x8 h, l; };
__device__ __forceinline__ APair apair_load(const float* cur, int blk, int lane) { return APair{lds_h(cur, blk, lane), lds_h(cur, blk + 1, lane)}; }
__device__ __forceinline__ void apair_pin(APair& a) {
    typedef unsigned u32x4 __attribute__((ext_vector_type(4)));
    u32x4 x = __builtin_bit_cast(u32x4, a.h), y = __builtin_bit_cast(u32x4, a.l);
    asm volatile("" : "+v"(x), "+v"(y));
    a.h = __builtin_bit_cast(f16x8, x); a.l = __builtin_bit_cast(f16x8, y);
}
__device__ __forceinline__ void apipe_step(APair& curp, APair& nextp, const float* cur, int next_blk, int lane) {
    apair_pin(curp);
    if (next_blk >= 0) nextp = apair_load(cur, next_blk, lane);
    __builtin_amdgcn_sched_barrier(0);
}

template <int KSI, int NCTO, int NT, int F, bool BN, int CH0, int NEXT_NBLK, int WG = OWH_WG, bool HOUT = false, bool REM2 = false, int NS = 2, bool AP = false>
__device__ __forceinline__ void conv_mel_hx(const Op (&in)[NT][KSI], f32x4 (&out)[NT][NCTO], const WRing<NS>& ring,
                                            const float* __restrict__ w, const float* __restrict__ w_next,
                                            const float* __restrict__ init, float cl, int wave, int lane,
                                            lanemask_t& bad) {
    using namespace owr;
    const int pos = lane & 15, j = lane >> 4;
    constexpr int SH = kInterleave ? 16 / F : 1;
    constexpr bool MASKS = F < 16 && !kInterleave;
    const bool first = (pos & (F - 1)) == 0, last = (pos & (F - 1)) == F - 1;
    constexpr int NBLK = 3 * KSI * 2;
#pragma unroll
    for (int oct = 0; oct < NCTO; ++oct) {
        const float* cur = ring_begin<NS, CH0, NBLK, NCTO, NEXT_NBLK, WG>(ring, oct, w, w_next, wave, lane);
        f32x4 res[NT], accs[2][NT];
        APair ap[2];
        if constexpr (AP) ap[0] = apair_load(cur, 0, lane);
#pragma unroll
        for (int ti = 0; ti < 3; ++ti) {
            const int tap = ti == 0 ? 0 : (ti == 1 ? 2 : 1);
            f32x4 acc[NT];
            f32x4 I = {0.f, 0.f, 0.f, 0.f};
            if (ti == 2) I = acc_init(BN ? init : nullptr, oct, j);
#pragma unroll
            for (int t = 0; t < NT; ++t) {
                if (ti < 2) acc[t] = f32x4{0.f, 0.f, 0.f, 0.f};
                else {
#pragma unroll
                    for (int e = 0; e < 4; ++e) {
                        if (HOUT && oct == NCTO - 1 && e >= 2) { acc[t][e] = 0.f; continue; }
                        const float l = dpp_shr_zero<SH>(accs[0][t][e]);
                        acc[t][e] = unpaired<F>(I[e] + ((MASKS && first) ? 0.f : l));
                    }
                }
            }
#pragma unroll
            for (int ks = 0; ks < KSI; ++ks) {
                f16x8 ah, al;
                if constexpr (AP) {
                    const int g = ti * KSI + ks;
                    const int ntap = ks + 1 < KSI ? tap : (ti == 0 ? 2 : 1), nks = ks + 1 < KSI ? ks + 1 : 0;
                    apipe_step(ap[g & 1], ap[(g + 1) & 1], cur, g + 1 < 3 * KSI ? (ntap * KSI + nks) * 2 : -1, lane);
                    ah = ap[g & 1].h; al = ap[g & 1].l;
                } else {
                    ah = lds_h(cur, (tap * KSI + ks) * 2 + 0, lane);
                    al = lds_h(cur, (tap * KSI + ks) * 2 + 1, lane);
                }
                if (REM2 && ks == KSI - 1) {
#pragma unroll
                    for (int t = 0; t < NT; ++t) acc[t] = OWH_MFMA(ah, in[t][ks].l, acc[t]);
#pragma unroll
                    for (int t = 0; t < NT; ++t) acc[t] = OWH_MFMA(al, in[t][ks].h, acc[t]);
                    continue;
                }
#pragma unroll
                for (int t = 0; t < NT; ++t) acc[t] = OWH_MFMA(ah, in[t][ks].h, acc[t]);
#pragma unroll
                for (int t = 0; t < NT; ++t) acc[t] = OWH_MFMA(ah, in[t][ks].l, acc[t]);
#pragma unroll
                for (int t = 0; t < NT; ++t) acc[t] = OWH_MFMA(al, in[t][ks].h, acc[t]);
            }
#pragma unroll
            for (int t = 0; t < NT; ++t) {
                if (ti < 2) accs[ti][t] = acc[t];
                else {
#pragma unroll
                    for (int e = 0; e < 4; ++e) {
                        if (HOUT && oct == NCTO - 1 && e >= 2) { res[t][e] = 0.f; continue; }
                        const float hh = dpp_shl_zero<SH>(accs[1][t][e]);
                        res[t][e] = acc[t][e] + ((MASKS && last) ? 0.f : hh);
                    }
                }
            }
        }
        if (oct == 0) {
#pragma unroll
            for (int t = 0; t < NT; ++t) nan_guard(bad, res[t][0]);
        }
#pragma unroll
        for (int t = 0; t < NT; ++t) {
            if (HOUT && oct == NCTO - 1) { out[t][oct] = act_t<BN, true>(res[t], cl); pin_t<true>(out[t][oct]); }
            else { out[t][oct] = act_t<BN, false>(res[t], cl); pin_t<false>(out[t][oct]); }
        }
        ring_end<NS, NBLK, NCTO, NEXT_NBLK, WG>(oct);
    }
}

template <int KSI, int NT, int F, int NPR>
__device__ __forceinline__ void merge_mel_rems(const Op (&in)[NT][KSI], Op (&M)[NT][(3 * NPR + 3) / 4]) {
    typedef unsigned u32x4 __attribute__((ext_vector_type(4)));
    static_assert(kInterleave || F == 16, "the operand shift relies on the zero fill at the stream edges");
    constexpr int SH = 16 / F, NMK = (3 * NPR + 3) / 4;
#pragma unroll
    for (int t = 0; t < NT; ++t) {
        const u32x4 sh = __builtin_bit_cast(u32x4, in[t][KSI - 1].h), sl = __builtin_bit_cast(u32x4, in[t][KSI - 1].l);
        unsigned h[NMK * 4], l[NMK * 4];
#pragma unroll
        for (int i = 0; i < NMK * 4; ++i) {
            const int tap = i / NPR, v = i % NPR;
            if (i >= 3 * NPR) { h[i] = 0u; l[i] = 0u; }
            else if (tap == 0) { h[i] = __builtin_amdgcn_update_dpp(0, sh[v], 0x110 + SH, 0xf, 0xf, true); l[i] = __builtin_amdgcn_update_dpp(0, sl[v], 0x110 + SH, 0xf, 0xf, true); }
            else if (tap == 2) { h[i] = __builtin_amdgcn_update_dpp(0, sh[v], 0x100 + SH, 0xf, 0xf, true); l[i] = __builtin_amdgcn_update_dpp(0, sl[v], 0x100 + SH, 0xf, 0xf, true); }
            else { h[i] = sh[v]; l[i] = sl[v]; }
        }
#pragma unroll
        for (int mk = 0; mk < NMK; ++mk) {
            M[t][mk].h = __builtin_bit_cast(f16x8, u32x4{h[4 * mk], h[4 * mk + 1], h[4 * mk + 2], h[4 * mk + 3]});
            M[t][mk].l = __builtin_bit_cast(f16x8, u32x4{l[4 * mk], l[4 * mk + 1], l[4 * mk + 2], l[4 * mk + 3]});
            pin_op(M[t][mk]);
        }
    }
}
template <int KSI, int NMK, int NCTO, int NT, int F, bool BN, int CH0, int NEXT_NBLK, int WG = OWH_WG, bool HOUT = false, int NS = 2, bool AP = false>
__device__ __forceinline__ void conv_mel_hxm(const Op (&in)[NT][KSI], const Op (&M)[NT][NMK], f32x4 (&out)[NT][NCTO], const WRing<NS>& ring,
                                             const float* __restrict__ w, const float* __restrict__ w_next,
                                             const float* __restrict__ init, float cl, int wave, int lane,
                                             lanemask_t& bad) {
    using namespace owr;
    const int j = lane >> 4;
    constexpr int SH = 16 / F, KSF = KSI - 1;
    constexpr int NBLK = (3 * KSF + NMK) * 2;
#pragma unroll
    for (int oct = 0; oct < NCTO; ++oct) {
        const float* cur = ring_begin<NS, CH0, NBLK, NCTO, NEXT_NBLK, WG>(ring, oct, w, w_next, wave, lane);
        f32x4 res[NT], accs[2][NT];
        APair ap[2];
        if constexpr (AP) ap[0] = apair_load(cur, 0, lane);
        int g = 0;
#pragma unroll
        for (int ti = 0; ti < 3; ++ti) {
            const int tap = ti == 0 ? 0 : (ti == 1 ? 2 : 1);
            f32x4 acc[NT];
            f32x4 I = {0.f, 0.f, 0.f, 0.f};
            if (ti == 2) I = acc_init(BN ? init : nullptr, oct, j);
#pragma unroll
            for (int t = 0; t < NT; ++t) {
                if (ti < 2) acc[t] = f32x4{0.f, 0.f, 0.f, 0.f};
                else {
#pragma unroll
                    for (int e = 0; e < 4; ++e) {
                        if (HOUT && oct == NCTO - 1 && e >= 2) { acc[t][e] = 0.f; continue; }
                        acc[t][e] = unpaired<F>(I[e] + dpp_shr_zero<SH>(accs[0][t][e]));
                    }
                }
            }
#pragma unroll
            for (int ks = 0; ks < KSF + (ti == 2 ? NMK : 0); ++ks) {
                const int mk = ks < KSF ? 0 : ks - KSF;
                const int blk = ks < KSF ? (tap * KSF + ks) * 2 : (3 * KSF + mk) * 2;
                f16x8 ah, al;
                if constexpr (AP) {
                    const int nsteps = KSF + (ti == 2 ? NMK : 0);
                    int nblk = -1;
                    if (ks + 1 < nsteps) nblk = ks + 1 < KSF ? (tap * KSF + ks + 1) * 2 : (3 * KSF + (ks + 1 - KSF)) * 2;
                    else if (ti < 2) nblk = KSF > 0 ? ((ti == 0 ? 2 : 1) * KSF) * 2 : (3 * KSF) * 2;
                    apipe_step(ap[g & 1], ap[(g + 1) & 1], cur, nblk, lane);
                    ah = ap[g & 1].h; al = ap[g & 1].l;
                    ++g;
                } else {
                    ah = lds_h(cur, blk + 0, lane);
                    al = lds_h(cur, blk + 1, lane);
                }
#pragma unroll
                for (int t = 0; t < NT; ++t) acc[t] = OWH_MFMA(ah, ks < KSF ? in[t][ks].h : M[t][mk].h, acc[t]);
#pragma unroll
                for (int t = 0; t < NT; ++t) acc[t] = OWH_MFMA(ah, ks < KSF ? in[t][ks].l : M[t][mk].l, acc[t]);
#pragma unroll
                for (int t = 0; t < NT; ++t) acc[t] = OWH_MFMA(al, ks < KSF ? in[t][ks].h : M[t][mk].h, acc[t]);
            }
#pragma unroll
            for (int t = 0; t < NT; ++t) {
                if (ti < 2) accs[ti][t] = acc[t];
                else {
#pragma unroll
                    for (int e = 0; e < 4; ++e) {
                        if (HOUT && oct == NCTO - 1 && e >= 2) { res[t][e] = 0.f; continue; }
                        res[t][e] = acc[t][e] + dpp_shl_zero<SH>(accs[1][t][e]);
                    }
                }
            }
        }
        if (oct == 0) {
#pragma unroll
            for (int t = 0; t < NT; ++t) nan_guard(bad, res[t][0]);
        }
#pragma unroll
        for (int t = 0; t < NT; ++t) {
            if (HOUT && oct == NCTO - 1) { out[t][oct] = act_t<BN, true>(res[t], cl); pin_t<true>(out[t][oct]); }
            else { out[t][oct] = act_t<BN, false>(res[t], cl); pin_t<false>(out[t][oct]); }
        }
        ring_end<NS, NBLK, NCTO, NEXT_NBLK, WG>(oct);
    }
}

#ifndef OWH_PIPE
#define OWH_PIPE 1
#endif
#ifndef OWH_PIPE_VALU
#define OWH_PIPE_VALU 2
#endif
#ifndef OWH_PIPE_M
#define OWH_PIPE_M 0
#endif
template <int KSI, int NCTO, int NR, bool BN, int CH0, int NEXT_NBLK, int WG = OWH_WG, bool GUARD = true, bool HOUT = false, bool PIPE = OWH_PIPE != 0, bool REM2 = false, int NS = 2, bool AP = false>
__device__ __forceinline__ void conv_time_hx(const Op (&h0)[KSI], const Op (&h1)[KSI], const Op (&in)[NR][KSI], f32x4 (&out)[NR][NCTO],
                                             const WRing<NS>& ring, const float* __restrict__ w, const float* __restrict__ w_next,
                                             const float* __restrict__ init, float cl, int wave, int lane,
                                             lanemask_t& bad) {
    using namespace owr;
    const int j = lane >> 4;
    constexpr int NBLK = 3 * KSI * 2;
    f32x4 prev[NR];
#pragma unroll
    for (int oct = 0; oct <= NCTO; ++oct) {
        f32x4 acc[NR];
        if (oct < NCTO) {
            const float* cur = ring_begin<NS, CH0, NBLK, NCTO, NEXT_NBLK, WG>(ring, oct, w, w_next, wave, lane);
            const f32x4 I = acc_init(BN ? init : nullptr, oct, j);
#pragma unroll
            for (int r = 0; r < NR; ++r) acc[r] = I;
            APair ap[2];
            if constexpr (AP) ap[0] = apair_load(cur, 0, lane);
#pragma unroll
            for (int tap = 0; tap < 3; ++tap)
#pragma unroll
                for (int ks = 0; ks < KSI; ++ks) {
                    f16x8 ah, al;
                    if constexpr (AP) {
                        const int g = tap * KSI + ks;
                        apipe_step(ap[g & 1], ap[(g + 1) & 1], cur, g + 1 < 3 * KSI ? (g + 1) * 2 : -1, lane);
                        ah = ap[g & 1].h; al = ap[g & 1].l;
                    } else {
                        ah = lds_h(cur, (tap * KSI + ks) * 2 + 0, lane);
                        al = lds_h(cur, (tap * KSI + ks) * 2 + 1, lane);
                    }
                    const bool rem = REM2 && ks == KSI - 1;
#pragma unroll
                    for (int part = 0; part < (rem ? 2 : 3); ++part)
#pragma unroll
                        for (int r = 0; r < NR; ++r) {
                            const int src = r + tap;
                            const int ri = src >= 2 ? src - 2 : 0;
                            const Op& b = src == 0 ? h0[ks] : (src == 1 ? h1[ks] : in[ri][ks]);
                            if (rem) acc[r] = OWH_MFMA(part == 0 ? ah : al, part == 0 ? b.l : b.h, acc[r]);
                            else acc[r] = OWH_MFMA(part == 2 ? al : ah, part == 1 ? b.l : b.h, acc[r]);
                        }
                }
        }
        if (oct > 0) {
            if (GUARD && oct == 1) {
#pragma unroll
                for (int r = 0; r < NR; ++r) nan_guard(bad, prev[r][0]);
            }
#pragma unroll
            for (int r = 0; r < NR; ++r) {
                if (HOUT && oct == NCTO) { out[r][oct - 1] = act_t<BN, true>(prev[r], cl); pin_t<true>(out[r][oct - 1]); }
                else { out[r][oct - 1] = act_t<BN, false>(prev[r], cl); pin_t<false>(out[r][oct - 1]); }
            }
        }
        if (PIPE && !AP && oct > 0 && oct < NCTO) {
#pragma unroll
            for (int i = 0; i < (9 * KSI - (REM2 ? 3 : 0)) * NR; ++i) {
                __builtin_amdgcn_sched_group_barrier(0x008, 1, 0);
                __builtin_amdgcn_sched_group_barrier(0x002, OWH_PIPE_VALU, 0);
            }
        }
        if (oct < NCTO) {
#pragma unroll
            for (int r = 0; r < NR; ++r) prev[r] = acc[r];
                ring_end<NS, NBLK, NCTO, NEXT_NBLK, WG>(oct);
        }
    }
}

template <int NCT, bool HALF> struct TimeK {
    static constexpr int KSF = NCT / 2;
    static constexpr int NPR = NCT % 2 ? (HALF ? 1 : 2) : 0;
    static constexpr int NMK = (3 * NPR + 3) / 4;
    static constexpr int NBLK = (3 * KSF + NMK) * 2;
};

struct RemPairs { unsigned h[2], l[2]; };
template <int NCT, bool HALF>
__device__ __forceinline__ void to_ops_time(const f32x4 (&t)[NCT], Op (&full)[TimeK<NCT, HALF>::KSF], RemPairs& rem) {
    typedef unsigned u32x4 __attribute__((ext_vector_type(4)));
#pragma unroll
    for (int k = 0; k < NCT / 2; ++k) { full[k] = split_pair(t[2 * k], t[2 * k + 1]); pin_op(full[k]); }
    const Op o = split_some<TimeK<NCT, HALF>::NPR>(t[NCT - 1], f32x4{0.f, 0.f, 0.f, 0.f});
    const u32x4 oh = __builtin_bit_cast(u32x4, o.h), ol = __builtin_bit_cast(u32x4, o.l);
#pragma unroll
    for (int v = 0; v < 2; ++v) { rem.h[v] = v < TimeK<NCT, HALF>::NPR ? oh[v] : 0u; rem.l[v] = v < TimeK<NCT, HALF>::NPR ? ol[v] : 0u; }
}
template <int NR, int NPR, int NMK>
__device__ __forceinline__ void merge_rems(const RemPairs (&rem)[NR + 2], Op (&M)[NR][NMK]) {
    typedef unsigned u32x4 __attribute__((ext_vector_type(4)));
#pragma unroll
    for (int r = 0; r < NR; ++r) {
        unsigned h[NMK * 4], l[NMK * 4];
#pragma unroll
        for (int i = 0; i < NMK * 4; ++i) {
            const int tap = i / NPR, v = i % NPR;
            h[i] = i < 3 * NPR ? rem[r + (tap < 3 ? tap : 0)].h[v] : 0u;
            l[i] = i < 3 * NPR ? rem[r + (tap < 3 ? tap : 0)].l[v] : 0u;
        }
#pragma unroll
        for (int mk = 0; mk < NMK; ++mk) {
            M[r][mk].h = __builtin_bit_cast(f16x8, u32x4{h[4 * mk], h[4 * mk + 1], h[4 * mk + 2], h[4 * mk + 3]});
            M[r][mk].l = __builtin_bit_cast(f16x8, u32x4{l[4 * mk], l[4 * mk + 1], l[4 * mk + 2], l[4 * mk + 3]});
            pin_op(M[r][mk]);
        }
    }
}

template <int KSF, int NMK, int NCTO, int NR, bool BN, int CH0, int NEXT_NBLK, int WG = OWH_WG, bool HOUT = false, int NS = 2, bool AP = false>
__device__ __forceinline__ void conv_time_hxm(const Op (&h0)[KSF], const Op (&h1)[KSF], const Op (&in)[NR][KSF], const Op (&M)[NR][NMK],
                                              f32x4 (&out)[NR][NCTO], const WRing<NS>& ring, const float* __restrict__ w, const float* __restrict__ w_next,
                                              const float* __restrict__ init, float cl, int wave, int lane,
                                              lanemask_t& bad) {
    using namespace owr;
    const int j = lane >> 4;
    constexpr int NBLK = (3 * KSF + NMK) * 2;
    f32x4 prev[NR];
#pragma unroll
    for (int oct = 0; oct <= NCTO; ++oct) {
        f32x4 acc[NR];
        if (oct < NCTO) {
            const float* cur = ring_begin<NS, CH0, NBLK, NCTO, NEXT_NBLK, WG>(ring, oct, w, w_next, wave, lane);
            const f32x4 I = acc_init(BN ? init : nullptr, oct, j);
#pragma unroll
            for (int r = 0; r < NR; ++r) acc[r] = I;
            APair ap[2];
            if constexpr (AP) ap[0] = apair_load(cur, 0, lane);
#pragma unroll
            for (int tap = 0; tap < 3; ++tap)
#pragma unroll
                for (int ks = 0; ks < KSF; ++ks) {
                    f16x8 ah, al;
                    if constexpr (AP) {
                        const int g = tap * KSF + ks;
                        apipe_step(ap[g & 1], ap[(g + 1) & 1], cur, g + 1 < 3 * KSF + NMK ? (g + 1) * 2 : -1, lane);
                        ah = ap[g & 1].h; al = ap[g & 1].l;
                    } else {
                        ah = lds_h(cur, (tap * KSF + ks) * 2 + 0, lane);
                        al = lds_h(cur, (tap * KSF + ks) * 2 + 1, lane);
                    }
#pragma unroll
                    for (int part = 0; part < 3; ++part)
#pragma unroll
                        for (int r = 0; r < NR; ++r) {
                            const int src = r + tap;
                            const int ri = src >= 2 ? src - 2 : 0;
                            const Op& b = src == 0 ? h0[ks] : (src == 1 ? h1[ks] : in[ri][ks]);
                            acc[r] = OWH_MFMA(part == 2 ? al : ah, part == 1 ? b.l : b.h, acc[r]);
                        }
                }
#pragma unroll
            for (int mk = 0; mk < NMK; ++mk) {
                f16x8 ah, al;
                if constexpr (AP) {
                    const int g = 3 * KSF + mk;
                    apipe_step(ap[g & 1], ap[(g + 1) & 1], cur, g + 1 < 3 * KSF + NMK ? (g + 1) * 2 : -1, lane);
                    ah = ap[g & 1].h; al = ap[g & 1].l;
                } else {
                    ah = lds_h(cur, (3 * KSF + mk) * 2 + 0, lane);
                    al = lds_h(cur, (3 * KSF + mk) * 2 + 1, lane);
                }
#pragma unroll
                for (int part = 0; part < 3; ++part)
#pragma unroll
                    for (int r = 0; r < NR; ++r) acc[r] = OWH_MFMA(part == 2 ? al : ah, part == 1 ? M[r][mk].l : M[r][mk].h, acc[r]);
            }
        }
        if (oct > 0) {
            if (oct == 1) {
#pragma unroll
                for (int r = 0; r < NR; ++r) nan_guard(bad, prev[r][0]);
            }
#pragma unroll
            for (int r = 0; r < NR; ++r) {
                if (HOUT && oct == NCTO) { out[r][oct - 1] = act_t<BN, true>(prev[r], cl); pin_t<true>(out[r][oct - 1]); }
                else { out[r][oct - 1] = act_t<BN, false>(prev[r], cl); pin_t<false>(out[r][oct - 1]); }
            }
        }
#if OWH_PIPE_M
        if (oct > 0 && oct < NCTO) {
#pragma unroll
            for (int i = 0; i < 3 * (3 * KSF + NMK) * NR; ++i) {
                __builtin_amdgcn_sched_group_barrier(0x008, 1, 0);
                __builtin_amdgcn_sched_group_barrier(0x002, OWH_PIPE_VALU, 0);
            }
        }
#endif
        if (oct < NCTO) {
#pragma unroll
            for (int r = 0; r < NR; ++r) prev[r] = acc[r];
                ring_end<NS, NBLK, NCTO, NEXT_NBLK, WG>(oct);
        }
    }
}

#ifndef OWH_HIST_LDS
#define OWH_HIST_LDS 1
#endif
#ifndef OWH_HIST_LDS_C
#define OWH_HIST_LDS_C 0
#endif
#ifndef OWH_SPRIO_B
#define OWH_SPRIO_B 1111
#endif
#ifndef OWH_SPRIO_RB
#define OWH_SPRIO_RB 1223
#endif
#ifndef OWH_RES_HIST_EARLY
#define OWH_RES_HIST_EARLY 0
#endif
#ifndef OWH_SPRIO_C
#define OWH_SPRIO_C 3210
#endif
#ifndef OWH_SPRIO_D
#define OWH_SPRIO_D 3210
#endif
#ifndef OWH_SPRIO_E
#define OWH_SPRIO_E 1111
#endif
template <int CODE, int LAYER> __device__ __forceinline__ void sprio() {
    constexpr int div = LAYER == 0 ? 1000 : LAYER == 1 ? 100 : LAYER == 2 ? 10 : 1;
    if constexpr (CODE != 0 && LAYER >= 0) __builtin_amdgcn_s_setprio((CODE / div) % 10);
    if constexpr (CODE != 0 && LAYER < 0) __builtin_amdgcn_s_setprio(0);
}
template <int NBLK>
__device__ __forceinline__ void issue_hist(const float* __restrict__ gsrc, float* ldst, int lane) {
    const float* base = owr::uniform_ptr(gsrc);
#pragma unroll
    for (int i = 0; i < NBLK; ++i)
        __builtin_amdgcn_global_load_lds((const __attribute__((address_space(1))) void*)(base + i * 256 + lane * 4),
                                         (__attribute__((address_space(3))) void*)(ldst + i * 256), 16, 0, 0);
}
template <int NCT, bool HALF>
__device__ __forceinline__ void load_tile_lds(f32x4 (&t)[NCT], const float* base, int lane) {
#pragma unroll
    for (int ct = 0; ct < NCT; ++ct)
#pragma unroll
        for (int e = 0; e < 4; ++e) {
            if (HALF && ct == NCT - 1 && e >= 2) t[ct][e] = 0.f;
            else t[ct][e] = base[(ct * 4 + e) * 64 + lane];
        }
}

constexpr int RES_B_WG = 12, RES_B_LDS_BYTES = 126 * 1024;
template <bool RES> __device__ __forceinline__ float* res_lds(float* ring_slot0) {
    if constexpr (RES) { extern __shared__ __attribute__((aligned(16))) float res_dyn[]; return res_dyn; }
    else return ring_slot0;
}
template <class C, bool LAST, bool DBG, int WG = OWH_WG, int NS = 2>
__global__ __launch_bounds__(64 * WG, (DBG || NS > 3 || NS == 1 ? 1 : (NS == 3 && C::WPS > 2 ? 2 : C::WPS))) void hstage_kernel(owr::RStageParams p) {
    using namespace owr;
    constexpr int NCTI = C::NCTI, NCT = C::NCT, R = C::RP, F = C::F;
    static_assert(!LAST || C::NPASS == 1, "the last stage runs in one pass");
    static_assert(NS == 2 || C::NPASS == 1 || (4 * NCT) % NS == 0, "multi-pass stages need a ring phase that returns to 0 after each pass");
    static_assert(NS >= 1 && NS <= 5 && NS - 1 <= NCT, "the chunks in flight at a layer boundary belong to at most the next layer");
    constexpr bool RES = NS == 1;
    static_assert(!RES || (!LAST && !DBG && C::NPASS == 1), "resident weights: one pass, no debug dumps, not the last stage");
    constexpr int KSA = (NCTI + 1) / 2, KS = (NCT + 1) / 2;
    constexpr int NBA = 3 * KSA * 2, NB = 3 * KS * 2;
    using TK = TimeK<NCT, C::HOUT>;
    constexpr bool MERGE = OWH_KMERGE && (NCT % 2 == 1) && !LAST && (C::HOUT || OWH_KMERGE_B);
    constexpr int NBT = MERGE ? TK::NBLK : NB;
    constexpr bool PIPE = OWH_PIPE != 0;
    constexpr int APCFG = NCT == 3 ? OWH_APIPE_B : NCT == 5 ? OWH_APIPE_C : LAST ? OWH_APIPE_E : OWH_APIPE_D;
    constexpr bool APM = (APCFG & 1) != 0, APT = (APCFG & 2) != 0;
    constexpr int SPCODE = NS == 1 ? OWH_SPRIO_RB : NCT == 3 ? OWH_SPRIO_B : NCT == 5 ? OWH_SPRIO_C : LAST ? OWH_SPRIO_E : OWH_SPRIO_D;
    constexpr bool REM2 = OWH_REM2 && NCT % 2 == 1 && !C::HOUT && !LAST && !(OWH_KMERGE && OWH_KMERGE_B) && !(OWH_KMERGE_MEL && OWH_KMERGE_MEL2B);
    constexpr bool MMA2 = OWH_KMERGE_MEL && OWH_KMERGE_MEL2 && kInterleave && !C::HIN && NCTI % 2 == 1 && NCTI >= 3 && C::WPS == 2;
    constexpr bool MMA = (OWH_KMERGE_MEL && kInterleave && C::HIN && NCTI % 2 == 1 && NCTI >= 3) || MMA2;
    constexpr int NPRA = MMA2 ? 2 : 1, NMKA = (3 * NPRA + 3) / 4;
    constexpr bool MMC2 = OWH_KMERGE_MEL && OWH_KMERGE_MEL2B && !C::HOUT && NCT % 2 == 1 && NCT >= 3 && !LAST;
    constexpr bool MMC = (OWH_KMERGE_MEL && kInterleave && C::HOUT && NCT % 2 == 1 && NCT >= 3) || MMC2;
    constexpr int NPRC = MMC2 ? 2 : 1, NMKC = (3 * NPRC + 3) / 4;
    constexpr int NBAM = MMA ? (3 * (KSA - 1) + NMKA) * 2 : NBA, NBCM = MMC ? (3 * (KS - 1) + NMKC) * 2 : NB;
    constexpr int NBMAX = (NBAM > NBT ? NBAM : NBT) > (NBCM > (LAST ? NB : 0) ? NBCM : (LAST ? NB : 0)) ? (NBAM > NBT ? NBAM : NBT) : (NBCM > (LAST ? NB : 0) ? NBCM : (LAST ? NB : 0));
    constexpr int WBS = NBMAX * 256;
    constexpr bool HLDS = OWH_HIST_LDS && !RES && !LAST && C::NPASS == 1 && (C::SPT == 1 || (C::SPT == 2 && OWH_HIST_LDS_C));
    constexpr int HROW = NCT * 4 * 64;
    const int lane0 = threadIdx.x & 63;
    const int wave = __builtin_amdgcn_readfirstlane(threadIdx.x >> 6);
    int g = blockIdx.x * WG + wave;
    __shared__ __attribute__((aligned(16))) float wbuf[RES ? 4 : WBS];
    __shared__ __attribute__((aligned(16))) float wbuf1[RES ? 4 : WBS];
    __shared__ __attribute__((aligned(16))) float wbuf2[NS >= 3 ? WBS : 4];
    __shared__ __attribute__((aligned(16))) float wbuf3[NS >= 4 ? WBS : 4];
    __shared__ __attribute__((aligned(16))) float wbuf4[NS >= 5 ? WBS : 4];
    constexpr int RES_OFF_B = NCT * NBAM * 256, RES_OFF_C = RES_OFF_B + NCT * NBT * 256, RES_OFF_D = RES_OFF_C + NCT * NBCM * 256;
    static_assert(!RES || (RES_OFF_D + NCT * NBT * 256) * 4 == RES_B_LDS_BYTES, "launch_rstage sizes the dynamic LDS with RES_B_LDS_BYTES");
    float* const rw = res_lds<RES>(wbuf);
    const WRing<NS> ring{{rw, RES ? rw + RES_OFF_B : wbuf1, RES ? rw + RES_OFF_C : wbuf2, RES ? rw + RES_OFF_D : wbuf3, wbuf4}};
    __shared__ __attribute__((aligned(16))) float sbn[4][NCT * 16];
    __shared__ __attribute__((aligned(16))) float hlds[HLDS ? WG * 2 * HROW : 4];
    float* const hl = hlds + (HLDS ? wave * 2 * HROW : 0);
    __shared__ int res_next;
    const bool active = RES || g < p.n_groups;
    int g_end = 0;
    if constexpr (RES) {
        const int nwg = gridDim.x, per = p.n_groups / nwg, rem = p.n_groups % nwg, b = blockIdx.x;
        const int g_lo = b * per + min(b, rem);
        g_end = g_lo + per + (b < rem ? 1 : 0);
        if (threadIdx.x == 0) res_next = g_lo;
        constexpr int off4[5] = {0, RES_OFF_B / 4, RES_OFF_C / 4, RES_OFF_D / 4, RES_B_LDS_BYTES / 16};
        constexpr int NT = 64 * WG, MAXU = (off4[2] - off4[1] + NT - 1) / NT;
        static_assert(off4[1] <= MAXU * NT && off4[3] - off4[2] <= MAXU * NT && off4[4] - off4[3] <= MAXU * NT, "layer b's array is the largest");
        f32x4 t[4][MAXU];
#pragma unroll
        for (int l = 0; l < 4; ++l)
#pragma unroll
            for (int u = 0; u < MAXU; ++u) {
                const int i = threadIdx.x + u * NT;
                if (i < off4[l + 1] - off4[l]) t[l][u] = reinterpret_cast<const f32x4*>(p.w[l])[i];
            }
#pragma unroll
        for (int l = 0; l < 4; ++l)
#pragma unroll
            for (int u = 0; u < MAXU; ++u) {
                const int i = threadIdx.x + u * NT;
                if (i < off4[l + 1] - off4[l]) reinterpret_cast<f32x4*>(rw)[off4[l] + i] = t[l][u];
            }
    } else {
    if (!active) g = p.n_groups - 1;
    if (p.glist) g = p.glist[g];
    else g += p.g_base;
    }
    lanemask_t bad = 0;
    if constexpr (!RES) {
    ring_issue<NS, NBAM, WG>(p.w[0], wbuf, wave, lane0);
    if (NS >= 3) ring_issue<NS, NBAM, WG>(p.w[0] + (size_t)NBAM * 256, wbuf1, wave, lane0);
    if (NS >= 4) ring_issue<NS, NBAM, WG>(p.w[0] + (size_t)2 * NBAM * 256, wbuf2, wave, lane0);
    if (NS >= 5) ring_issue<NS, NBAM, WG>(p.w[0] + (size_t)3 * NBAM * 256, wbuf3, wave, lane0);
    }
    for (int i = threadIdx.x; i < 4 * NCT * 16; i += 64 * WG) {
        const int l = i / (NCT * 16), c = i % (NCT * 16);
        sbn[l][c] = p.shift[l][c];
    }
    if constexpr (RES) __syncthreads();
    for (;;) {
    int lane_z = 0;
    if constexpr (RES) asm volatile("" : "+v"(lane_z));
    const int lane = RES ? ((lane0 + lane_z) & 63) : lane0;
    if constexpr (RES) {
        int k = 0;
        if (lane0 == 0) k = __hip_atomic_fetch_add(&res_next, 1, __ATOMIC_RELAXED, __HIP_MEMORY_SCOPE_WORKGROUP);
        g = __builtin_amdgcn_readfirstlane(k);
        if (g >= g_end) break;
        g += p.g_base;
        bad = 0;
    }
    const int s_first = g * C::SPT;
    const bool lane_on = active && (p.stream_on == nullptr || p.stream_on[min(s_first + tile_stream<F>(lane & 15), p.S - 1)] != 0);
    float* hb = p.hist_b + (size_t)g * C::HIST_FLOATS;
    float* hd = p.hist_d + (size_t)g * C::HIST_FLOATS;
    if (HLDS) issue_hist<2 * NCT>(hb, hl, lane);

#pragma unroll
    for (int pass = 0; pass < C::NPASS; ++pass) {
    f32x4 Y[R][NCT];
    Op Xo[R][KSA];
#pragma unroll
    for (int r = 0; r < R; ++r) {
        f32x4 X[NCTI];
        load_tile_h<NCTI, C::HIN>(X, p.xin + ((size_t)price_alias<(OWH_PRICE_HANDOVER & 2) != 0 && C::CIN == 24>(g) * C::R + pass * R + r) * (NCTI * 4 * 64), lane);
        to_ops<NCTI, C::HIN>(X, Xo[r]);
    }
    constexpr bool HEARLY = RES && OWH_RES_HIST_EARLY != 0 && !MERGE;
    f32x4 E0[HEARLY ? NCT : 1], E1[HEARLY ? NCT : 1];
    if constexpr (HEARLY) { load_tile_h<NCT, C::HOUT>(E0, hb, lane); load_tile_h<NCT, C::HOUT>(E1, hb + NCT * 4 * 64, lane); }
    if (!RES && pass == 0) chunk_sync();
    sprio<SPCODE, 0>();

    if constexpr (MMA) {
        Op Mx[R][NMKA];
        merge_mel_rems<KSA, R, F, NPRA>(Xo, Mx);
        conv_mel_hxm<KSA, NMKA, NCT, R, F, true, 0, NBT, WG, C::HOUT, NS, APM>(Xo, Mx, Y, ring, p.w[0], p.w[1], sbn[0], p.clampv[0], wave, lane, bad);
    } else
    conv_mel_hx<KSA, NCT, R, F, true, 0, NBT, WG, C::HOUT, false, NS, APM>(Xo, Y, ring, p.w[0], p.w[1], sbn[0], p.clampv[0], wave, lane, bad);
    if (DBG && p.dbg && active) {
#pragma unroll
        for (int r = 0; r < R; ++r) dump_tile_ht<NCT, F, C::C>(Y[r], p.dbg, p.dbg_stride, p.dbg_off[0], s_first, pass * R + r, p.S, lane, p.dbg_mul[0]);
    }
    Op Ao[R][KS], H0[KS], H1[KS];
    sprio<SPCODE, 1>();
    if constexpr (MERGE) {
        Op AoF[R][TK::KSF], H0F[TK::KSF], H1F[TK::KSF], M[R][TK::NMK];
        RemPairs rem[R + 2];
        {
            f32x4 T0[NCT], T1[NCT];
            if (HLDS) { load_tile_lds<NCT, C::HOUT>(T0, hl, lane); load_tile_lds<NCT, C::HOUT>(T1, hl + HROW, lane); }
            else { load_tile_h<NCT, C::HOUT>(T0, hb, lane); load_tile_h<NCT, C::HOUT>(T1, hb + NCT * 4 * 64, lane); }
            to_ops_time<NCT, C::HOUT>(T0, H0F, rem[0]);
            to_ops_time<NCT, C::HOUT>(T1, H1F, rem[1]);
        }
        if (HLDS) { asm volatile("s_waitcnt lgkmcnt(0)" ::: "memory"); issue_hist<2 * NCT>(hd, hl, lane); }
        if (lane_on) {
            store_tile_h<NCT, C::HOUT>(Y[R - 2], hb, lane);
            store_tile_h<NCT, C::HOUT>(Y[R - 1], hb + NCT * 4 * 64, lane);
        }
#pragma unroll
        for (int r = 0; r < R; ++r) to_ops_time<NCT, C::HOUT>(Y[r], AoF[r], rem[2 + r]);
        merge_rems<R, TK::NPR, TK::NMK>(rem, M);
        __builtin_amdgcn_sched_barrier(0);
        conv_time_hxm<TK::KSF, TK::NMK, NCT, R, true, NCT, NBCM, WG, C::HOUT, NS, APT>(H0F, H1F, AoF, M, Y, ring, p.w[1], p.w[2], sbn[1], p.clampv[1], wave, lane, bad);
    } else {
    if constexpr (HEARLY) { to_ops<NCT, C::HOUT, REM2>(E0, H0); to_ops<NCT, C::HOUT, REM2>(E1, H1); }
    else {
        f32x4 T0[NCT], T1[NCT];
        if (HLDS) { load_tile_lds<NCT, C::HOUT>(T0, hl, lane); load_tile_lds<NCT, C::HOUT>(T1, hl + HROW, lane); }
        else { load_tile_h<NCT, C::HOUT>(T0, hb, lane); load_tile_h<NCT, C::HOUT>(T1, hb + NCT * 4 * 64, lane); }
        to_ops<NCT, C::HOUT, REM2>(T0, H0);
        to_ops<NCT, C::HOUT, REM2>(T1, H1);
    }
    if (HLDS) { asm volatile("s_waitcnt lgkmcnt(0)" ::: "memory"); issue_hist<2 * NCT>(hd, hl, lane); }
    if (lane_on) {
        store_tile_h<NCT, C::HOUT>(Y[R - 2], hb, lane);
        store_tile_h<NCT, C::HOUT>(Y[R - 1], hb + NCT * 4 * 64, lane);
    }
#pragma unroll
    for (int r = 0; r < R; ++r) to_ops<NCT, C::HOUT, REM2>(Y[r], Ao[r]);
    __builtin_amdgcn_sched_barrier(0);
    conv_time_hx<KS, NCT, R, true, NCT, NBCM, WG, true, C::HOUT, PIPE, REM2, NS, APT>(H0, H1, Ao, Y, ring, p.w[1], p.w[2], sbn[1], p.clampv[1], wave, lane, bad);
    }
    if (DBG && p.dbg && active) {
#pragma unroll
        for (int r = 0; r < R; ++r) dump_tile_ht<NCT, F, C::C>(Y[r], p.dbg, p.dbg_stride, p.dbg_off[1], s_first, pass * R + r, p.S, lane, p.dbg_mul[1]);
    }
#pragma unroll
    for (int r = 0; r < R; ++r) to_ops<NCT, C::HOUT, REM2>(Y[r], Ao[r]);
    __builtin_amdgcn_sched_barrier(0);
    if constexpr (HEARLY) { load_tile_h<NCT, C::HOUT>(E0, hd, lane); load_tile_h<NCT, C::HOUT>(E1, hd + NCT * 4 * 64, lane); }
    sprio<SPCODE, 2>();
    if constexpr (MMC) {
        Op Mc[R][NMKC];
        merge_mel_rems<KS, R, F, NPRC>(Ao, Mc);
        conv_mel_hxm<KS, NMKC, NCT, R, F, true, 2 * NCT, NBT, WG, C::HOUT, NS, APM>(Ao, Mc, Y, ring, p.w[2], p.w[3], sbn[2], p.clampv[2], wave, lane, bad);
    } else
    conv_mel_hx<KS, NCT, R, F, true, 2 * NCT, NBT, WG, C::HOUT, REM2, NS, APM>(Ao, Y, ring, p.w[2], p.w[3], sbn[2], p.clampv[2], wave, lane, bad);
    if (DBG && p.dbg && active) {
#pragma unroll
        for (int r = 0; r < R; ++r) dump_tile_ht<NCT, F, C::C>(Y[r], p.dbg, p.dbg_stride, p.dbg_off[2], s_first, pass * R + r, p.S, lane, p.dbg_mul[2]);
    }
    sprio<SPCODE, 3>();
    if constexpr (MERGE) {
        Op AoF[R][TK::KSF], H0F[TK::KSF], H1F[TK::KSF], M[R][TK::NMK];
        RemPairs rem[R + 2];
        {
            f32x4 T0[NCT], T1[NCT];
            if (HLDS) { load_tile_lds<NCT, C::HOUT>(T0, hl, lane); load_tile_lds<NCT, C::HOUT>(T1, hl + HROW, lane); }
            else { load_tile_h<NCT, C::HOUT>(T0, hd, lane); load_tile_h<NCT, C::HOUT>(T1, hd + NCT * 4 * 64, lane); }
            to_ops_time<NCT, C::HOUT>(T0, H0F, rem[0]);
            to_ops_time<NCT, C::HOUT>(T1, H1F, rem[1]);
        }
        if (lane_on) {
            store_tile_h<NCT, C::HOUT>(Y[R - 2], hd, lane);
            store_tile_h<NCT, C::HOUT>(Y[R - 1], hd + NCT * 4 * 64, lane);
        }
#pragma unroll
        for (int r = 0; r < R; ++r) to_ops_time<NCT, C::HOUT>(Y[r], AoF[r], rem[2 + r]);
        merge_rems<R, TK::NPR, TK::NMK>(rem, M);
        __builtin_amdgcn_sched_barrier(0);
        conv_time_hxm<TK::KSF, TK::NMK, NCT, R, true, 3 * NCT, (C::NPASS > 1 ? NBAM : 0), WG, C::HOUT, NS, APT>(H0F, H1F, AoF, M, Y, ring, p.w[3], p.w[0], sbn[3], p.clampv[3], wave, lane, bad);
    } else {
    if constexpr (HEARLY) { to_ops<NCT, C::HOUT, REM2>(E0, H0); to_ops<NCT, C::HOUT, REM2>(E1, H1); }
    else {
        f32x4 T0[NCT], T1[NCT];
        if (HLDS) { load_tile_lds<NCT, C::HOUT>(T0, hl, lane); load_tile_lds<NCT, C::HOUT>(T1, hl + HROW, lane); }
        else { load_tile_h<NCT, C::HOUT>(T0, hd, lane); load_tile_h<NCT, C::HOUT>(T1, hd + NCT * 4 * 64, lane); }
        to_ops<NCT, C::HOUT, REM2>(T0, H0);
        to_ops<NCT, C::HOUT, REM2>(T1, H1);
    }
    if (lane_on) {
        store_tile_h<NCT, C::HOUT>(Y[R - 2], hd, lane);
        store_tile_h<NCT, C::HOUT>(Y[R - 1], hd + NCT * 4 * 64, lane);
    }
#pragma unroll
    for (int r = 0; r < R; ++r) to_ops<NCT, C::HOUT, REM2>(Y[r], Ao[r]);
    __builtin_amdgcn_sched_barrier(0);
    conv_time_hx<KS, NCT, R, true, 3 * NCT, (LAST ? NB : (C::NPASS > 1 ? NBAM : 0)), WG, true, C::HOUT, PIPE, REM2, NS, APT>(H0, H1, Ao, Y, ring, p.w[3], LAST ? p.w19 : p.w[0], sbn[3], p.clampv[3], wave, lane, bad);
    }
    if (DBG && p.dbg && active) {
#pragma unroll
        for (int r = 0; r < R; ++r) dump_tile_ht<NCT, F, C::C>(Y[r], p.dbg, p.dbg_stride, p.dbg_off[3], s_first, pass * R + r, p.S, lane, p.dbg_mul[3]);
    }

    sprio<SPCODE, -1>();
    if (!LAST && lane_on) {
        constexpr int FO = C::FO, RO = C::RO;
        constexpr int SPTN = 16 / FO;
        const int pos = lane & 15, j = lane >> 4;
        const int sp = tile_stream<F>(pos), f = tile_mel<F>(pos);
        const int s = g * C::SPT + sp;
        const int gn = s / SPTN, spn = s % SPTN;
        const int posn = tile_pos<FO>(spn, f / 2);
        constexpr int SH = kInterleave ? C::SPT : 1;
#pragma unroll
        for (int ro = 0; ro < R / C::PT; ++ro) {
            float pm[NCT][4];
#pragma unroll
            for (int ct = 0; ct < NCT; ++ct)
#pragma unroll
                for (int e = 0; e < 4; ++e) {
                    if (C::HOUT && ct == NCT - 1 && e >= 2) { pm[ct][e] = 0.f; continue; }
                    float m = Y[ro * C::PT][ct][e];
                    if (C::PT == 2) m = fmax_nc(m, Y[ro * C::PT + 1][ct][e]);
                    pm[ct][e] = fmax_nc(m, dpp_shl_zero<SH>(m)) * p.xmul;
                }
            if ((f & 1) == 0) {
                float* xo = p.xout + ((size_t)(gn * RO + pass * (R / C::PT) + ro) * (NCT * 4)) * 64 + j * 16 + posn;
#pragma unroll
                for (int ct = 0; ct < NCT; ++ct)
#pragma unroll
                    for (int e = 0; e < 4; ++e)
                        if (!(C::HOUT && ct == NCT - 1 && e >= 2)) xo[(ct * 4 + e) * 64] = pm[ct][e];
            }
        }
    }
    if (LAST) {
        static_assert(!LAST || (C::RO == 1 && C::FO == 1 && NCT == 6), "last stage pools to one position, 96 channels");
        const int pos = lane & 15, j = lane >> 4;
        f32x4 Pl[NCT];
        const int src = (j * 16 + tile_pos<F>(pos & 7, 0)) * 4;
        constexpr int SH = kInterleave ? C::SPT : 1;
#pragma unroll
        for (int ct = 0; ct < NCT; ++ct)
#pragma unroll
            for (int e = 0; e < 4; ++e) {
                float m = fmax_nc(Y[0][ct][e], Y[1][ct][e]);
                m = fmax_nc(m, dpp_shl_zero<SH>(m)) * p.xmul;
                Pl[ct][e] = __builtin_bit_cast(float, __builtin_amdgcn_ds_bpermute(src, __builtin_bit_cast(int, m)));
            }
        float* h19 = p.hist19 + (size_t)g * (2 * NCT * 4 * 64);
        f32x4 T0[NCT], T1[NCT];
        Op H0[KS], H1[KS];
        load_tile<NCT>(T0, h19, lane);
        load_tile<NCT>(T1, h19 + NCT * 4 * 64, lane);
        to_ops<NCT>(T0, H0);
        to_ops<NCT>(T1, H1);
        Op Po[1][KS];
        to_ops<NCT>(Pl, Po[0]);
        f32x4 E[1][NCT];
        conv_time_hx<KS, NCT, 1, false, 4 * NCT, 0, WG, false, false, OWH_PIPE != 0, false, NS>(H0, H1, Po, E, ring, p.w19, nullptr, nullptr, 0.f, wave, lane, bad);
        const bool on19 = active && (p.stream_on == nullptr || p.stream_on[min(s_first + (pos & 7), p.S - 1)] != 0);
        if (on19) {
            store_tile<NCT>(T1, h19, lane);
            store_tile<NCT>(Pl, h19 + NCT * 4 * 64, lane);
        }
        const int s = s_first + pos;
        if (on19 && pos < C::SPT && s < p.S) {
            const uint32_t slot = p.nfeat[s] % (uint32_t)p.TR;
#pragma unroll
            for (int ct = 0; ct < NCT; ++ct) {
                const f32x4 ev = E[0][ct] * p.emb_mul;
                *reinterpret_cast<f32x4*>(p.feat + ((size_t)s * p.TR + slot) * 96 + ct * 16 + 4 * j) = ev;
                *reinterpret_cast<f32x4*>(p.emb + (size_t)s * 96 + ct * 16 + 4 * j) = ev;
                if (DBG && p.dbg) *reinterpret_cast<f32x4*>(p.dbg + (size_t)s * p.dbg_stride + p.dbg_off[4] + ct * 16 + 4 * j) = ev;
            }
        }
    }
    }
    if (!LAST && C::NPASS > 1) asm volatile("s_waitcnt vmcnt(0)" ::: "memory");
    if (bad != 0) {
        if (lane0 == 0) {
            float* hb0 = p.hist_b + (size_t)g * C::HIST_FLOATS;
            for (int q = 0; q < 16; ++q) if ((bad >> q) & 1) hb0[q] = __builtin_nanf("");
        }
        raise_range_flag(bad, p.range_flag, s_first, C::SPT);
    }
    if constexpr (!RES) break;
    }
}

#ifndef OWF_QPRIO
#if !defined(OWF_PRIO) || OWF_PRIO == 6
#define OWF_QPRIO 2233
#else
#define OWF_QPRIO 0
#endif
#endif
namespace sa {
constexpr int RS = 34;
constexpr int PLANE = 344;
constexpr int WAVE_HALVES = 2 * PLANE;
}
typedef unsigned u32x4 __attribute__((ext_vector_type(4)));

__device__ __forceinline__ void stageA_fill_gather_table(int* gtab , int tid, int nt) {
    for (int i = tid; i < 512; i += nt) {
        const int lane = i >> 3, q = i & 7, p = lane & 15, g = lane >> 4, slot = 8 * g + q;
        const int tap = slot % 9, plane = slot >= 18 ? 1 : 0;
        gtab[i] = slot < 27 ? 2 * (plane * sa::PLANE + (tap / 3) * sa::RS + (tap % 3) + 2 * p) : 0;
    }
}
__device__ __forceinline__ void stageA_put_mel(_Float16* sP, int row, int bin, float v) {
    const _Float16 hi = (_Float16)v;
    sP[row * sa::RS + 1 + bin] = hi;
    sP[sa::PLANE + row * sa::RS + 1 + bin] = (_Float16)(v - (float)hi);
}
__device__ __forceinline__ f32x4 mfma3(const f16x8 ah, const f16x8 al, const Op& x, f32x4 c) {
    c = OWH_MFMA(ah, x.h, c);
    c = OWH_MFMA(ah, x.l, c);
    return OWH_MFMA(al, x.h, c);
}
__device__ __forceinline__ void dump_tile_a(const f32x4 (&t)[2], float* __restrict__ dbg, size_t stride, int off, int s, int row, int h,
                                            int S, int lane, float mul) {
    if (s >= S) return;
    const int pos = lane & 15, j = lane >> 4;
#pragma unroll
    for (int ct = 0; ct < 2; ++ct)
#pragma unroll
        for (int e = 0; e < 4; ++e) {
            const int c = ct == 0 ? 4 * j + e : (e < 2 ? 16 + 2 * j + e : 24);
            if (c < 24) dbg[(size_t)s * stride + off + (row * 32 + 2 * pos + h) * 24 + c] = t[ct][e] * mul;
        }
}
// ... 1060 lines not shown
```

Measured before the change: 24.28 million frames/s.

## Add half-resident LDS weight mode for stage C with streamed low halves

Adds a persistent-grid launch path for stage C (HC) that keeps only the high f16 halves of the split weights resident in LDS (130 KB). The low halves are streamed from global memory through a per-lane register look-ahead queue inside the A-operand pipeline. The goal is to remove the per-chunk LDS ring refills and barriers for stage C when the group count is large, which it is at this stream count. The cost is extra global or L2 traffic for the low halves, higher register pressure from the queue, and one workgroup per CU of occupancy.

```diff
diff --git a/openwakeword_amd/csrc/owwhip.hip b/openwakeword_amd/csrc/owwhip.hip
--- a/openwakeword_amd/csrc/owwhip.hip
+++ b/openwakeword_amd/csrc/owwhip.hip
@@ -156,6 +156,8 @@
 constexpr int kSmallLaunchWgs = 2 * 256;
 constexpr int kResidentBMinGroups = 8192;
 constexpr int kResidentBWgs = 256;
+constexpr int kResidentCMinGroups = 32768;
+constexpr int kResidentCWgs = 256;
 
 struct FastGroup : HeadGroup {
     DevBuf<NetDesc> d_nets;
@@ -264,6 +266,7 @@
     std::vector<int16_t> cal_user;
     int small_wgs = kSmallLaunchWgs, small_wgs_heads = kSmallLaunchWgs;
     int resident_b = -1, resident_b_wgs = kResidentBWgs;
+    int resident_c = -1, resident_c_wgs = kResidentCWgs;
     float hx_selftest_err = 0.f, hx_selftest_ref = 0.f, hx_selftest_score_err = 0.f;
     bool fuse = false;
     DevBuf<float> d_verw, d_verb, d_verthr; DevBuf<int> d_verT;
@@ -442,6 +445,14 @@
             return;
         }
     }
+    if constexpr (HX && !DBG && std::is_same<CH, owh::HC>::value) {
+        const bool resident = p.glist == nullptr && p.n_groups > 0 && (h->resident_c < 0 ? p.n_groups >= kResidentCMinGroups : h->resident_c != 0);
+        if (resident) {
+            const int grid = std::max(1, std::min(h->resident_c_wgs, (p.n_groups + owh::RES_C_WG - 1) / owh::RES_C_WG));
+            hipLaunchKernelGGL((owh::hstage_kernel<CH, LAST, false, owh::RES_C_WG, 0>), dim3(grid), dim3(64 * owh::RES_C_WG), owh::RES_C_LDS_BYTES, st, p);
+            return;
+        }
+    }
     if (HX && !DBG && nwg <= h->small_wgs) hipLaunchKernelGGL((owh::hstage_kernel<CH, LAST, false, WG, 3>), dim3(nwg), dim3(64 * WG), 0, st, p);
     else if (HX) hipLaunchKernelGGL((owh::hstage_kernel<CH, LAST, DBG, WG>), dim3(nwg), dim3(64 * WG), 0, st, p);
     else hipLaunchKernelGGL((owr::rstage_kernel<CR, LAST, DBG>), dim3((p.n_groups + 3) / 4), dim3(256), 0, st, p);
@@ -1359,6 +1370,7 @@
     if (h->vad) lds(owv::vad_front_kernel, owv::V_LDS_BYTES);
     lds(owf::hmelA_kernel<false>, owf::FA_LDS_BYTES); lds(owf::hmelA_kernel<true>, owf::FA_LDS_BYTES);
     lds(owh::hstage_kernel<owh::HB, false, false, owh::RES_B_WG, 1>, owh::RES_B_LDS_BYTES);
+    lds(owh::hstage_kernel<owh::HC, false, false, owh::RES_C_WG, 0>, owh::RES_C_LDS_BYTES);
     lds(stageA_kernel<true>, CfgA::LDS_BYTES); lds(stageA_kernel<false>, CfgA::LDS_BYTES);
     lds(stage_kernel<CfgB, true, false>, CfgB::LDS_BYTES); lds(stage_kernel<CfgB, false, false>, CfgB::LDS_BYTES);
     lds(stage_kernel<CfgC, true, false>, CfgC::LDS_BYTES); lds(stage_kernel<CfgC, false, false>, CfgC::LDS_BYTES);
@@ -2091,6 +2103,8 @@
     if (const char* e = getenv("OWW_SMALL_WGS_HEADS")) h->small_wgs_heads = atoi(e);
     if (const char* e = getenv("OWW_RESIDENT_B")) h->resident_b = strcmp(e, "auto") == 0 ? -1 : (atoi(e) != 0 ? 1 : 0);
     if (const char* e = getenv("OWW_RESIDENT_B_WGS")) h->resident_b_wgs = std::max(1, atoi(e));
+    if (const char* e = getenv("OWW_RESIDENT_C")) h->resident_c = strcmp(e, "auto") == 0 ? -1 : (atoi(e) != 0 ? 1 : 0);
+    if (const char* e = getenv("OWW_RESIDENT_C_WGS")) h->resident_c_wgs = std::max(1, atoi(e));
     if (const char* e = getenv("OWW_GENERIC_SPW")) { const int v = atoi(e); h->generic_spw = v == 4 || v == 16 ? v : 0; }
     h->post_in_heads = h->fuse && h->groups.size() == 1 && h->groups[0].ht == 4 && h->generic_nets.empty() && h->rnn_nets.empty() && h->NL > 0;
     if (int rc = set_kernel_lds(h)) return rc;
diff --git a/openwakeword_amd/csrc/owwhip_hx.h b/openwakeword_amd/csrc/owwhip_hx.h
--- a/openwakeword_amd/csrc/owwhip_hx.h
+++ b/openwakeword_amd/csrc/owwhip_hx.h
@@ -277,7 +277,11 @@
 template <int NS, int CH, int NBLK, int NCTO, int NEXT_NBLK, int WG>
 __device__ __forceinline__ const float* ring_begin(const WRing<NS>& r, int oct, const float* __restrict__ w, const float* __restrict__ w_next,
                                                    int wave, int lane) {
-    if constexpr (NS == 1) {
+    if constexpr (NS == 0) {
+        int z = 0;
+        asm volatile("" : "+s"(z));
+        return r.s[CH / NCTO] + oct * (NBLK / 2) * 256 + z;
+    } else if constexpr (NS == 1) {
         int z = 0;
         asm volatile("" : "+s"(z));
         return r.s[CH / NCTO] + oct * NBLK * 256 + z;
@@ -292,8 +296,8 @@
 }
 template <int NS, int NBLK, int NCTO, int NEXT_NBLK, int WG>
 __device__ __forceinline__ void ring_end(int oct) {
-    if (NS == 1 || !(oct + 1 < NCTO || NEXT_NBLK > 0)) return;
-    if constexpr (NS == 1) {}
+    if (NS <= 1 || !(oct + 1 < NCTO || NEXT_NBLK > 0)) return;
+    if constexpr (NS <= 1) {}
     else if constexpr (NS == 2) owr::chunk_sync();
     else {
         constexpr int P = NS - 1, A = (NBLK + WG - 1) / WG, B = NEXT_NBLK > 0 ? ((NEXT_NBLK > 0 ? NEXT_NBLK : 1) + WG - 1) / WG : 0;
@@ -328,6 +332,44 @@
 __device__ __forceinline__ void apipe_step(APair& curp, APair& nextp, const float* cur, int next_blk, int lane) {
     apair_pin(curp);
     if (next_blk >= 0) nextp = apair_load(cur, next_blk, lane);
+    __builtin_amdgcn_sched_barrier(0);
+}
+
+#ifndef OWH_RESC_DEPTH
+#define OWH_RESC_DEPTH 4
+#endif
+template <int QD> struct LoQ { f16x8 q[QD > 0 ? QD : 1]; };
+__device__ __forceinline__ f16x8 lo_load(const float* __restrict__ src, int lane) {
+    return *(const __attribute__((address_space(1))) f16x8*)(src + (unsigned)(lane * 4));
+}
+constexpr int mel_group_blk(int KSF, int NMK, int g) {
+    return g < KSF ? g * 2 : g < 2 * KSF ? (KSF + g) * 2 : g < 3 * KSF ? (g - KSF) * 2 : g * 2;
+}
+struct LoSrc { const float* w; int off; bool on; };
+template <int QD, int NG, int NBLK, int NCTO, bool MEL, int KSF, int NMK, bool NEXT, int NKSF, int NNMK>
+__device__ __forceinline__ LoSrc lo_ahead(const float* __restrict__ w, const float* __restrict__ w_next, int oct, int g) {
+    static_assert(QD <= NG, "the look-ahead reaches at most the next chunk");
+    int t = g + QD, c = oct;
+    if (t >= NG) { t -= NG; ++c; }
+    if (c < NCTO) return LoSrc{w, (c * NBLK + (MEL ? mel_group_blk(KSF, NMK, t) : 2 * t) + 1) * 256, true};
+    if (!NEXT) return LoSrc{w, 0, false};
+    return LoSrc{w_next, ((MEL ? 2 * t : mel_group_blk(NKSF, NNMK, t)) + 1) * 256, true};
+}
+#ifndef OWH_RESC_HI_AHEAD
+#define OWH_RESC_HI_AHEAD 1
+#endif
+template <int QD>
+__device__ __forceinline__ void apipe_step_hl(APair& curp, APair& nextp, const float* cur, int cur_hblk, int next_hblk, LoQ<QD>& q, int slot,
+                                              const LoSrc lo, int lane) {
+    curp.l = q.q[slot];
+    if (!OWH_RESC_HI_AHEAD && cur_hblk > 0) curp.h = lds_h(cur, cur_hblk, lane);
+    apair_pin(curp);
+    if (OWH_RESC_HI_AHEAD && next_hblk >= 0) nextp.h = lds_h(cur, next_hblk, lane);
+    if (lo.on) {
+        unsigned zoff = (unsigned)lo.off * 4u;
+        asm volatile("" : "+s"(zoff));
+        q.q[slot] = lo_load(reinterpret_cast<const float*>(reinterpret_cast<const char*>(lo.w) + zoff), lane);
+    }
     __builtin_amdgcn_sched_barrier(0);
 }
 
@@ -443,21 +485,23 @@
         }
     }
 }
-template <int KSI, int NMK, int NCTO, int NT, int F, bool BN, int CH0, int NEXT_NBLK, int WG = OWH_WG, bool HOUT = false, int NS = 2, bool AP = false>
+template <int KSI, int NMK, int NCTO, int NT, int F, bool BN, int CH0, int NEXT_NBLK, int WG = OWH_WG, bool HOUT = false, int NS = 2, bool AP = false, int QD = 0, int QB = 0>
 __device__ __forceinline__ void conv_mel_hxm(const Op (&in)[NT][KSI], const Op (&M)[NT][NMK], f32x4 (&out)[NT][NCTO], const WRing<NS>& ring,
                                              const float* __restrict__ w, const float* __restrict__ w_next,
                                              const float* __restrict__ init, float cl, int wave, int lane,
-                                             lanemask_t& bad) {
+                                             lanemask_t& bad, LoQ<QD>* loq = nullptr) {
     using namespace owr;
     const int j = lane >> 4;
     constexpr int SH = 16 / F, KSF = KSI - 1;
     constexpr int NBLK = (3 * KSF + NMK) * 2;
+    static_assert(NS != 0 || AP, "hi-resident weights come through the A-operand pipeline");
 #pragma unroll
     for (int oct = 0; oct < NCTO; ++oct) {
         const float* cur = ring_begin<NS, CH0, NBLK, NCTO, NEXT_NBLK, WG>(ring, oct, w, w_next, wave, lane);
         f32x4 res[NT], accs[2][NT];
         APair ap[2];
-        if constexpr (AP) ap[0] = apair_load(cur, 0, lane);
+        if constexpr (AP && NS == 0) ap[0].h = lds_h(cur, 0, lane);
+        else if constexpr (AP) ap[0] = apair_load(cur, 0, lane);
         int g = 0;
 #pragma unroll
         for (int ti = 0; ti < 3; ++ti) {
@@ -486,6 +530,11 @@
                     int nblk = -1;
                     if (ks + 1 < nsteps) nblk = ks + 1 < KSF ? (tap * KSF + ks + 1) * 2 : (3 * KSF + (ks + 1 - KSF)) * 2;
                     else if (ti < 2) nblk = KSF > 0 ? ((ti == 0 ? 2 : 1) * KSF) * 2 : (3 * KSF) * 2;
+                    if constexpr (NS == 0) {
+                        constexpr int NG = 3 * KSF + NMK;
+                        apipe_step_hl<QD>(ap[g & 1], ap[(g + 1) & 1], cur, blk / 2, nblk < 0 ? -1 : nblk / 2, *loq, (QB + oct * NG + g) % QD,
+                                          lo_ahead<QD, NG, NBLK, NCTO, true, KSF, NMK, (NEXT_NBLK > 0), 0, 0>(w, w_next, oct, g), lane);
+                    } else
                     apipe_step(ap[g & 1], ap[(g + 1) & 1], cur, nblk, lane);
                     ah = ap[g & 1].h; al = ap[g & 1].l;
                     ++g;
@@ -644,14 +693,17 @@
     }
 }
 
-template <int KSF, int NMK, int NCTO, int NR, bool BN, int CH0, int NEXT_NBLK, int WG = OWH_WG, bool HOUT = false, int NS = 2, bool AP = false>
+template <int KSF, int NMK, int NCTO, int NR, bool BN, int CH0, int NEXT_NBLK, int WG = OWH_WG, bool HOUT = false, int NS = 2, bool AP = false,
+          int QD = 0, int QB = 0, int NKSF = 0, int NNMK = 0>
 __device__ __forceinline__ void conv_time_hxm(const Op (&h0)[KSF], const Op (&h1)[KSF], const Op (&in)[NR][KSF], const Op (&M)[NR][NMK],
                                               f32x4 (&out)[NR][NCTO], const WRing<NS>& ring, const float* __restrict__ w, const float* __restrict__ w_next,
                                               const float* __restrict__ init, float cl, int wave, int lane,
-                                              lanemask_t& bad) {
+                                              lanemask_t& bad, LoQ<QD>* loq = nullptr) {
     using namespace owr;
     const int j = lane >> 4;
     constexpr int NBLK = (3 * KSF + NMK) * 2;
+    static_assert(NS != 0 || AP, "hi-resident weights come through the A-operand pipeline");
+    constexpr int NG = 3 * KSF + NMK;
     f32x4 prev[NR];
 #pragma unroll
     for (int oct = 0; oct <= NCTO; ++oct) {
@@ -662,7 +714,8 @@
 #pragma unroll
             for (int r = 0; r < NR; ++r) acc[r] = I;
             APair ap[2];
-            if constexpr (AP) ap[0] = apair_load(cur, 0, lane);
+            if constexpr (AP && NS == 0) ap[0].h = lds_h(cur, 0, lane);
+            else if constexpr (AP) ap[0] = apair_load(cur, 0, lane);
 #pragma unroll
             for (int tap = 0; tap < 3; ++tap)
 #pragma unroll
@@ -670,6 +723,10 @@
                     f16x8 ah, al;
                     if constexpr (AP) {
                         const int g = tap * KSF + ks;
+                        if constexpr (NS == 0)
+                            apipe_step_hl<QD>(ap[g & 1], ap[(g + 1) & 1], cur, g, g + 1 < NG ? g + 1 : -1, *loq, (QB + oct * NG + g) % QD,
+                                              lo_ahead<QD, NG, NBLK, NCTO, false, 0, 0, (NEXT_NBLK > 0), NKSF, NNMK>(w, w_next, oct, g), lane);
+                        else
                         apipe_step(ap[g & 1], ap[(g + 1) & 1], cur, g + 1 < 3 * KSF + NMK ? (g + 1) * 2 : -1, lane);
                         ah = ap[g & 1].h; al = ap[g & 1].l;
                     } else {
@@ -691,6 +748,10 @@
                 f16x8 ah, al;
                 if constexpr (AP) {
                     const int g = 3 * KSF + mk;
+                    if constexpr (NS == 0)
+                        apipe_step_hl<QD>(ap[g & 1], ap[(g + 1) & 1], cur, g, g + 1 < NG ? g + 1 : -1, *loq, (QB + oct * NG + g) % QD,
+                                          lo_ahead<QD, NG, NBLK, NCTO, false, 0, 0, (NEXT_NBLK > 0), NKSF, NNMK>(w, w_next, oct, g), lane);
+                    else
                     apipe_step(ap[g & 1], ap[(g + 1) & 1], cur, g + 1 < 3 * KSF + NMK ? (g + 1) * 2 : -1, lane);
                     ah = ap[g & 1].h; al = ap[g & 1].l;
                 } else {
@@ -749,6 +810,9 @@
 #ifndef OWH_SPRIO_C
 #define OWH_SPRIO_C 3210
 #endif
+#ifndef OWH_SPRIO_RC
+#define OWH_SPRIO_RC 3210
+#endif
 #ifndef OWH_SPRIO_D
 #define OWH_SPRIO_D 3210
 #endif
@@ -780,18 +844,19 @@
 }
 
 constexpr int RES_B_WG = 12, RES_B_LDS_BYTES = 126 * 1024;
+constexpr int RES_C_WG = 8, RES_C_LDS_BYTES = 130 * 1024;
 template <bool RES> __device__ __forceinline__ float* res_lds(float* ring_slot0) {
     if constexpr (RES) { extern __shared__ __attribute__((aligned(16))) float res_dyn[]; return res_dyn; }
     else return ring_slot0;
 }
 template <class C, bool LAST, bool DBG, int WG = OWH_WG, int NS = 2>
-__global__ __launch_bounds__(64 * WG, (DBG || NS > 3 || NS == 1 ? 1 : (NS == 3 && C::WPS > 2 ? 2 : C::WPS))) void hstage_kernel(owr::RStageParams p) {
+__global__ __launch_bounds__(64 * WG, (DBG || NS > 3 || NS <= 1 ? 1 : (NS == 3 && C::WPS > 2 ? 2 : C::WPS))) void hstage_kernel(owr::RStageParams p) {
     using namespace owr;
     constexpr int NCTI = C::NCTI, NCT = C::NCT, R = C::RP, F = C::F;
     static_assert(!LAST || C::NPASS == 1, "the last stage runs in one pass");
     static_assert(NS == 2 || C::NPASS == 1 || (4 * NCT) % NS == 0, "multi-pass stages need a ring phase that returns to 0 after each pass");
-    static_assert(NS >= 1 && NS <= 5 && NS - 1 <= NCT, "the chunks in flight at a layer boundary belong to at most the next layer");
-    constexpr bool RES = NS == 1;
+    static_assert(NS >= 0 && NS <= 5 && NS - 1 <= NCT, "the chunks in flight at a layer boundary belong to at most the next layer");
+    constexpr bool HL = NS == 0, RES = NS <= 1;
     static_assert(!RES || (!LAST && !DBG && C::NPASS == 1), "resident weights: one pass, no debug dumps, not the last stage");
     constexpr int KSA = (NCTI + 1) / 2, KS = (NCT + 1) / 2;
     constexpr int NBA = 3 * KSA * 2, NB = 3 * KS * 2;
@@ -801,7 +866,7 @@
     constexpr bool PIPE = OWH_PIPE != 0;
     constexpr int APCFG = NCT == 3 ? OWH_APIPE_B : NCT == 5 ? OWH_APIPE_C : LAST ? OWH_APIPE_E : OWH_APIPE_D;
     constexpr bool APM = (APCFG & 1) != 0, APT = (APCFG & 2) != 0;
-    constexpr int SPCODE = NS == 1 ? OWH_SPRIO_RB : NCT == 3 ? OWH_SPRIO_B : NCT == 5 ? OWH_SPRIO_C : LAST ? OWH_SPRIO_E : OWH_SPRIO_D;
+    constexpr int SPCODE = NS == 0 ? OWH_SPRIO_RC : NS == 1 ? OWH_SPRIO_RB : NCT == 3 ? OWH_SPRIO_B : NCT == 5 ? OWH_SPRIO_C : LAST ? OWH_SPRIO_E : OWH_SPRIO_D;
     constexpr bool REM2 = OWH_REM2 && NCT % 2 == 1 && !C::HOUT && !LAST && !(OWH_KMERGE && OWH_KMERGE_B) && !(OWH_KMERGE_MEL && OWH_KMERGE_MEL2B);
     constexpr bool MMA2 = OWH_KMERGE_MEL && OWH_KMERGE_MEL2 && kInterleave && !C::HIN && NCTI % 2 == 1 && NCTI >= 3 && C::WPS == 2;
     constexpr bool MMA = (OWH_KMERGE_MEL && kInterleave && C::HIN && NCTI % 2 == 1 && NCTI >= 3) || MMA2;
@@ -822,8 +887,10 @@
     __shared__ __attribute__((aligned(16))) float wbuf2[NS >= 3 ? WBS : 4];
     __shared__ __attribute__((aligned(16))) float wbuf3[NS >= 4 ? WBS : 4];
     __shared__ __attribute__((aligned(16))) float wbuf4[NS >= 5 ? WBS : 4];
-    constexpr int RES_OFF_B = NCT * NBAM * 256, RES_OFF_C = RES_OFF_B + NCT * NBT * 256, RES_OFF_D = RES_OFF_C + NCT * NBCM * 256;
-    static_assert(!RES || (RES_OFF_D + NCT * NBT * 256) * 4 == RES_B_LDS_BYTES, "launch_rstage sizes the dynamic LDS with RES_B_LDS_BYTES");
+    constexpr int RES_DIV = HL ? 2 : 1, RES_BYTES = HL ? RES_C_LDS_BYTES : RES_B_LDS_BYTES;
+    constexpr int RES_OFF_B = NCT * NBAM * 256 / RES_DIV, RES_OFF_C = RES_OFF_B + NCT * NBT * 256 / RES_DIV, RES_OFF_D = RES_OFF_C + NCT * NBCM * 256 / RES_DIV;
+    static_assert(!RES || (RES_OFF_D + NCT * NBT * 256 / RES_DIV) * 4 == RES_BYTES, "launch_rstage sizes the dynamic LDS with RES_B_LDS_BYTES / RES_C_LDS_BYTES");
+    static_assert(!HL || (WG == RES_C_WG && MMA && MMC && MERGE && APM && APT), "hi resident: stage C, every layer K-merged and through the A-operand pipeline");
     float* const rw = res_lds<RES>(wbuf);
     const WRing<NS> ring{{rw, RES ? rw + RES_OFF_B : wbuf1, RES ? rw + RES_OFF_C : wbuf2, RES ? rw + RES_OFF_D : wbuf3, wbuf4}};
     __shared__ __attribute__((aligned(16))) float sbn[4][NCT * 16];
@@ -837,7 +904,7 @@
         const int g_lo = b * per + min(b, rem);
         g_end = g_lo + per + (b < rem ? 1 : 0);
         if (threadIdx.x == 0) res_next = g_lo;
-        constexpr int off4[5] = {0, RES_OFF_B / 4, RES_OFF_C / 4, RES_OFF_D / 4, RES_B_LDS_BYTES / 16};
+        constexpr int off4[5] = {0, RES_OFF_B / 4, RES_OFF_C / 4, RES_OFF_D / 4, RES_BYTES / 16};
         constexpr int NT = 64 * WG, MAXU = (off4[2] - off4[1] + NT - 1) / NT;
         static_assert(off4[1] <= MAXU * NT && off4[3] - off4[2] <= MAXU * NT && off4[4] - off4[3] <= MAXU * NT, "layer b's array is the largest");
         f32x4 t[4][MAXU];
@@ -846,7 +913,7 @@
 #pragma unroll
             for (int u = 0; u < MAXU; ++u) {
                 const int i = threadIdx.x + u * NT;
-                if (i < off4[l + 1] - off4[l]) t[l][u] = reinterpret_cast<const f32x4*>(p.w[l])[i];
+                if (i < off4[l + 1] - off4[l]) t[l][u] = reinterpret_cast<const f32x4*>(p.w[l])[HL ? ((i >> 6) << 7) + (i & 63) : i];
             }
 #pragma unroll
         for (int l = 0; l < 4; ++l)
@@ -884,6 +951,14 @@
         g += p.g_base;
         bad = 0;
     }
+    constexpr int QD = HL ? OWH_RESC_DEPTH : 0;
+    constexpr int NGA = 3 * (KSA - 1) + NMKA, NGT = 3 * TK::KSF + TK::NMK, NGC = 3 * (KS - 1) + NMKC;
+    LoQ<QD> loq;
+    if constexpr (HL) {
+        static_assert(QD >= 1 && QD <= NGA, "the queue is filled from conv a's first chunk");
+#pragma unroll
+        for (int i = 0; i < QD; ++i) loq.q[i] = lo_load(p.w[0] + (mel_group_blk(KSA - 1, NMKA, i) + 1) * 256, lane);
+    }
     const int s_first = g * C::SPT;
     const bool lane_on = active && (p.stream_on == nullptr || p.stream_on[min(s_first + tile_stream<F>(lane & 15), p.S - 1)] != 0);
     float* hb = p.hist_b + (size_t)g * C::HIST_FLOATS;
@@ -909,7 +984,7 @@
     if constexpr (MMA) {
         Op Mx[R][NMKA];
         merge_mel_rems<KSA, R, F, NPRA>(Xo, Mx);
-        conv_mel_hxm<KSA, NMKA, NCT, R, F, true, 0, NBT, WG, C::HOUT, NS, APM>(Xo, Mx, Y, ring, p.w[0], p.w[1], sbn[0], p.clampv[0], wave, lane, bad);
+        conv_mel_hxm<KSA, NMKA, NCT, R, F, true, 0, NBT, WG, C::HOUT, NS, APM, QD, 0>(Xo, Mx, Y, ring, p.w[0], p.w[1], sbn[0], p.clampv[0], wave, lane, bad, &loq);
     } else
     conv_mel_hx<KSA, NCT, R, F, true, 0, NBT, WG, C::HOUT, false, NS, APM>(Xo, Y, ring, p.w[0], p.w[1], sbn[0], p.clampv[0], wave, lane, bad);
     if (DBG && p.dbg && active) {
@@ -937,7 +1012,7 @@
         for (int r = 0; r < R; ++r) to_ops_time<NCT, C::HOUT>(Y[r], AoF[r], rem[2 + r]);
         merge_rems<R, TK::NPR, TK::NMK>(rem, M);
         __builtin_amdgcn_sched_barrier(0);
-        conv_time_hxm<TK::KSF, TK::NMK, NCT, R, true, NCT, NBCM, WG, C::HOUT, NS, APT>(H0F, H1F, AoF, M, Y, ring, p.w[1], p.w[2], sbn[1], p.clampv[1], wave, lane, bad);
+        conv_time_hxm<TK::KSF, TK::NMK, NCT, R, true, NCT, NBCM, WG, C::HOUT, NS, APT, QD, NCT * NGA, KS - 1, NMKC>(H0F, H1F, AoF, M, Y, ring, p.w[1], p.w[2], sbn[1], p.clampv[1], wave, lane, bad, &loq);
     } else {
     if constexpr (HEARLY) { to_ops<NCT, C::HOUT, REM2>(E0, H0); to_ops<NCT, C::HOUT, REM2>(E1, H1); }
     else {
@@ -969,7 +1044,7 @@
     if constexpr (MMC) {
         Op Mc[R][NMKC];
         merge_mel_rems<KS, R, F, NPRC>(Ao, Mc);
-        conv_mel_hxm<KS, NMKC, NCT, R, F, true, 2 * NCT, NBT, WG, C::HOUT, NS, APM>(Ao, Mc, Y, ring, p.w[2], p.w[3], sbn[2], p.clampv[2], wave, lane, bad);
+        conv_mel_hxm<KS, NMKC, NCT, R, F, true, 2 * NCT, NBT, WG, C::HOUT, NS, APM, QD, NCT * (NGA + NGT)>(Ao, Mc, Y, ring, p.w[2], p.w[3], sbn[2], p.clampv[2], wave, lane, bad, &loq);
     } else
     conv_mel_hx<KS, NCT, R, F, true, 2 * NCT, NBT, WG, C::HOUT, REM2, NS, APM>(Ao, Y, ring, p.w[2], p.w[3], sbn[2], p.clampv[2], wave, lane, bad);
     if (DBG && p.dbg && active) {
@@ -995,7 +1070,7 @@
         for (int r = 0; r < R; ++r) to_ops_time<NCT, C::HOUT>(Y[r], AoF[r], rem[2 + r]);
         merge_rems<R, TK::NPR, TK::NMK>(rem, M);
         __builtin_amdgcn_sched_barrier(0);
-        conv_time_hxm<TK::KSF, TK::NMK, NCT, R, true, 3 * NCT, (C::NPASS > 1 ? NBAM : 0), WG, C::HOUT, NS, APT>(H0F, H1F, AoF, M, Y, ring, p.w[3], p.w[0], sbn[3], p.clampv[3], wave, lane, bad);
+        conv_time_hxm<TK::KSF, TK::NMK, NCT, R, true, 3 * NCT, (C::NPASS > 1 ? NBAM : 0), WG, C::HOUT, NS, APT, QD, NCT * (NGA + NGT + NGC)>(H0F, H1F, AoF, M, Y, ring, p.w[3], p.w[0], sbn[3], p.clampv[3], wave, lane, bad, &loq);
     } else {
     if constexpr (HEARLY) { to_ops<NCT, C::HOUT, REM2>(E0, H0); to_ops<NCT, C::HOUT, REM2>(E1, H1); }
     else {
```

Result: no change. 24.37 million frames/s (median of 6 runs) (+0.4%).
